# HKU-BAL/ClairS-TO

Measured on AMD Instinct MI355X. Metric: candidate sites/sec (pileup-tensor + AFF/NEG inference) at 1/2/4/8 MI355X, higher is better.
Workload: dtype f32; 1 GPU; ONT 50x synthetic pileups, SNV (K=4), 1M-site job cut into 4096-site chunks (BASELINE.json configs[1]); step = featurize(AFF+NEG) + CvT + BiGRU + posterior on one chunk; batch=4096, chunks_resident_per_gpu=16, min_bq_aff=20, pack_bytes_per_chunk=28614435, parallelism=sites sharded, 1 rank/GPU, weights=seeded random init (no pretrained weights offline)

## Files before the change

### clairs_to_amd/csrc/cvt_block.h

```cpp
#pragma once
#include "cvt_gemm.h"

namespace cto {

__host__ __device__ constexpr int emb_ps(int cin) { return cin > 0 ? ((cin - 4 + 15) / 16) * 16 + 4 : 0; }
__host__ __device__ constexpr int emb_kch(int cin) { return (3 * emb_ps(cin) + 15) / 16; }

template <int C, int W, int WKV, int TS>
struct CvtBlockGeom {
    static constexpr int R = TS * W, RKV = TS * WKV;
    static constexpr int MT = (R + 15) / 16, MTKV = (RKV + 15) / 16;
    static constexpr int RS = C + 4, QS = 68, HC = (4 * C < 128 ? 4 * C : 128), US = HC + 4;
    static constexpr int OFF_Y = 0;
    static constexpr int OFF_YKV = OFF_Y + MT * 16 * RS;
    static constexpr int OFF_Q = OFF_YKV + MTKV * 16 * RS;
    static constexpr int OFF_K = OFF_Q + MT * 16 * QS;
    static constexpr int OFF_V = OFF_K + MTKV * 16 * QS;
    static constexpr int OFF_END = OFF_V + MTKV * 16 * QS;
    static constexpr int SCRATCH = OFF_END - OFF_YKV;
    static constexpr int U_FLOATS = MT * 16 * US;
    static constexpr int TOTAL = OFF_END + (U_FLOATS > SCRATCH ? U_FLOATS - SCRATCH : 0);
    static constexpr size_t LDS_BYTES = size_t(TOTAL) * sizeof(float);
    static constexpr int TMP_FLOATS = OFF_END - OFF_Q;
    static constexpr int ALIAS = TOTAL - OFF_YKV;
    static constexpr int KCH1 = (W * RS + 15) / 16;
    static constexpr int emb_floats(int cin) { return (MT * 32 + 4) * emb_ps(cin); }
    static constexpr bool HEAD_OK = (TS == 16) && (64 + head_lds_floats(6) <= ALIAS);
};

template <int C, int W, int WKV, int TS>
__host__ __device__ constexpr bool MT_EXACT() { return (TS * W) % 16 == 0 && (TS * WKV) % 16 == 0; }

constexpr int CVT_BLOCK_THREADS = 512;
constexpr int CVT_WAVES = CVT_BLOCK_THREADS / 64;

template <int N>
struct ColOwn {
    static constexpr int TILES = N / 16;
    static constexpr int NOWN = TILES < CVT_WAVES ? TILES : CVT_WAVES;
    static constexpr int MSPLIT = CVT_WAVES / NOWN;
    static constexpr int NTW = TILES / NOWN;
    static_assert(TILES * 16 == N && CVT_WAVES % NOWN == 0 && NTW * NOWN == TILES, "unsupported GEMM width");
};
template <int MTx, int MSPLIT>
struct MSplit {
    static constexpr int MTG = (MTx + MSPLIT - 1) / MSPLIT;
    static constexpr int FULL = MTx / MTG;
    static constexpr int LAST = MTx - FULL * MTG;
};
struct TileSpan { int tile0, mbase, mcount; };
template <int N, int MTx>
__device__ __forceinline__ TileSpan tile_span(int wave) {
    using O = ColOwn<N>;
    constexpr int MTG = MSplit<MTx, O::MSPLIT>::MTG;
    const int mb = (wave / O::NOWN) * MTG;
    const int left = MTx - mb;
    return TileSpan{(wave % O::NOWN) * O::NTW, mb, left < 0 ? 0 : (left > MTG ? MTG : left)};
}
template <int N, int MTx, int KCH>
__device__ __forceinline__ void gemm_span(const TileSpan& sp, const float* A, int lda, const float* const (&wrow)[ColOwn<N>::NTW],
                                          const BPre<ColOwn<N>::NTW>& pre,
                                          f32x4 (&acc)[MSplit<MTx, ColOwn<N>::MSPLIT>::MTG][ColOwn<N>::NTW], int j, int kg) {
    using S = MSplit<MTx, ColOwn<N>::MSPLIT>;
    constexpr int NTW = ColOwn<N>::NTW;
    const float* A0 = A + sp.mbase * 16 * lda;
    if (ColOwn<N>::MSPLIT == 1 || sp.mcount == S::MTG) {
        gemm_lds<S::MTG, NTW, KCH>(A0, lda, wrow, pre, acc, j, kg);
    } else if constexpr (S::LAST > 0) {
        if (sp.mcount == S::LAST) {
            f32x4 (&sub)[S::LAST][NTW] = reinterpret_cast<f32x4 (&)[S::LAST][NTW]>(acc);
            gemm_lds<S::LAST, NTW, KCH>(A0, lda, wrow, pre, sub, j, kg);
        }
    }
}

template <int N, int MTx, int KCH, bool F16>
__device__ __forceinline__ void gemm_span_split(const TileSpan& sp, const float* A, int lda, int klo,
                                                const unsigned short* const (&wrow)[ColOwn<N>::NTW],
                                                const BPreS<ColOwn<N>::NTW>& pre,
                                                f32x4 (&acc)[MSplit<MTx, ColOwn<N>::MSPLIT>::MTG][ColOwn<N>::NTW], int j, int kg) {
    using S = MSplit<MTx, ColOwn<N>::MSPLIT>;
    constexpr int NTW = ColOwn<N>::NTW;
    const float* A0 = A + sp.mbase * 16 * lda;
    if (ColOwn<N>::MSPLIT == 1 || sp.mcount == S::MTG) {
        gemm_lds_split<S::MTG, NTW, KCH, F16>(A0, lda, klo, wrow, pre, acc, j, kg);
    } else if constexpr (S::LAST > 0) {
        if (sp.mcount == S::LAST) {
            f32x4 (&sub)[S::LAST][NTW] = reinterpret_cast<f32x4 (&)[S::LAST][NTW]>(acc);
            gemm_lds_split<S::LAST, NTW, KCH, F16>(A0, lda, klo, wrow, pre, sub, j, kg);
        }
    }
}

template <int C, int W, int WKV, int TS>
__host__ __device__ constexpr int cvt_blocks_per_cu() {
    return CvtBlockGeom<C, W, WKV, TS>::LDS_BYTES * 3 <= 160 * 1024 ? 3 : (CvtBlockGeom<C, W, WKV, TS>::LDS_BYTES * 2 <= 160 * 1024 ? 2 : 1);
}

template <int C, int W, int WKV, int TS, int CIN, bool HEAD, int SPLIT = 0>
__global__ __launch_bounds__(CVT_BLOCK_THREADS, (2 * cvt_blocks_per_cu<C, W, WKV, TS>())) void k_cvt_block(float* __restrict__ h, CvtStageParams sp,
                                                                                                            HeadTailParams hp, int heads, int B) {
    using G = CvtBlockGeom<C, W, WKV, TS>;
    constexpr bool SP = SPLIT != 0, F16 = SPLIT == 1;
    static_assert(!SP || (C % 64 == 0 && MT_EXACT<C, W, WKV, TS>()), "split GEMMs: 32-wide k chunks, 16-byte LayerNorm pieces, no pad rows");
    using WPtr = std::conditional_t<SP, const unsigned short*, const float*>;
    static_assert(CIN == 0 || G::emb_floats(CIN) <= G::ALIAS, "stage input tile does not fit the free LDS");
    static_assert(!HEAD || G::HEAD_OK, "classifier tail needs a 16-site tile and room for its scratch");
    static_assert(G::MT * 16 * G::RS <= G::TMP_FLOATS, "LayerNorm staging tile does not fit the q|k|v region");
    constexpr int NT = CVT_BLOCK_THREADS, NWV = CVT_WAVES;
    constexpr int R = G::R, MT = G::MT, MTKV = G::MTKV, RKV = G::RKV, RS = G::RS, QS = G::QS, HC = G::HC, US = G::US;
    static_assert(C % 16 == 0 && C <= 128 && NT % C == 0, "channel count must be 16, 32, 64 or 128");
    using OC = ColOwn<C>;
    using OQ = ColOwn<64>;
    using OKV = ColOwn<128>;
    using OF = ColOwn<HC>;
    constexpr int MGC = MSplit<MT, OC::MSPLIT>::MTG, MGQ = MSplit<MT, OQ::MSPLIT>::MTG, MGF = MSplit<MT, OF::MSPLIT>::MTG;
    constexpr int NTC = OC::NTW, NTF = OF::NTW;
    static_assert(OQ::NTW == 1 && OKV::NTW == 1 && OKV::MSPLIT == 1, "q / kv tiles: one column tile per wave");
    extern __shared__ __attribute__((aligned(16))) float smem[];
    float* sy = smem + G::OFF_Y;
    float* sykv = smem + G::OFF_YKV;
    float* sq = smem + G::OFF_Q;
    float* sk = smem + G::OFF_K;
    float* sv = smem + G::OFF_V;
    float* stmp = smem + G::OFF_Q;
    float* su = smem + G::OFF_YKV;

    const int tid = threadIdx.x, lane = tid & 63, wave = tid >> 6, j = lane & 15, kg = lane >> 4;
    const TileSpan spc = tile_span<C, MT>(wave), spq = tile_span<64, MT>(wave), spf = tile_span<HC, MT>(wave);
    const int site0 = blockIdx.x * TS;
    const int nsite = min(TS, B - site0);
    const int rows_valid = nsite * W;
    const int inner = heads * 64;
    float* hg = h + int64_t(site0) * W * C;
    int nstamp = 0;
    long long* const prof = sp.blk[0].prof;
    auto stamp = [&]() { if (prof && blockIdx.x == 0 && tid == 0 && nstamp < 250) prof[nstamp++] = clock64(); };
    stamp();
    const CvtBlockParams& pe = sp.blk[0];


    constexpr int KE_ = CIN > 0 ? emb_kch(CIN) : 1;
    const float* we_r[NTC];
    BPre<NTC> pre_e;
    if constexpr (CIN > 0) {
#pragma unroll
        for (int nt = 0; nt < NTC; ++nt) we_r[nt] = pe.wembp + int64_t(spc.tile0 + nt) * (KE_ * FRAG_CS) + 4 * lane;
        pre_e = prefetch_b<NTC, KE_>(we_r);
    }
    if constexpr (HEAD) {
        for (int i = tid; i < MT * 16; i += NT) *reinterpret_cast<float4*>(sy + i * RS + C) = make_float4(0.f, 0.f, 0.f, 0.f);
    }
    if constexpr (CIN == 0) {
        constexpr int NIT = (MT * 16 * (C / 4) + NT - 1) / NT;
        float4 stage[NIT];
#pragma unroll
        for (int q = 0; q < NIT; ++q) {
            const int i = tid + q * NT, r = i / (C / 4), c4 = (i - r * (C / 4)) * 4;
            stage[q] = (i < MT * 16 * (C / 4) && r < rows_valid) ? *reinterpret_cast<const float4*>(hg + r * C + c4) : make_float4(0.f, 0.f, 0.f, 0.f);
        }
#pragma unroll
        for (int q = 0; q < NIT; ++q) {
            const int i = tid + q * NT, r = i / (C / 4), c4 = (i - r * (C / 4)) * 4;
            if (i < MT * 16 * (C / 4)) *reinterpret_cast<float4*>(sy + r * RS + c4) = stage[q];
        }
        for (int i = tid; i < (MTKV * 16 - RKV) * RS; i += NT) sykv[RKV * RS + i] = 0.f;
    } else {
        constexpr int WIN = 2 * W - 1, PS = emb_ps(CIN), NPOS = MT * 32 + 4, VW = (CIN % 4 == 0) ? 4 : 2, SLOTS = PS / VW;
        static_assert(CIN % 2 == 0, "stage input channels must be even");
        float* sin = smem + G::OFF_YKV;
        const float* xg = pe.xin + int64_t(site0) * WIN * CIN;
        constexpr int NIT = (NPOS * SLOTS + NT - 1) / NT;
        float4 stage[NIT];
#pragma unroll
        for (int q = 0; q < NIT; ++q) {
            const int i = tid + q * NT;
            const int pp = i / SLOTS, c = (i - pp * SLOTS) * VW;
            const int s = pp / (2 * W), pos = pp - s * 2 * W - 1;
            const bool ok = i < NPOS * SLOTS && pos >= 0 && s < nsite && c < CIN;
            float4 v = make_float4(0.f, 0.f, 0.f, 0.f);
            if (ok) {
                if (pe.xraw) {
                    const short* src = pe.xraw + (int64_t(site0 + s) * WIN + pos) * CIN + c;
                    if constexpr (VW == 4) { const uint2 w = *reinterpret_cast<const uint2*>(src); v.x = __uint_as_float(w.x); v.y = __uint_as_float(w.y); }
                    else v.x = __uint_as_float(*reinterpret_cast<const unsigned*>(src));
                } else {
                    const float* src = xg + (s * WIN + pos) * CIN + c;
                    if constexpr (VW == 4) v = *reinterpret_cast<const float4*>(src);
                    else { const float2 w2 = *reinterpret_cast<const float2*>(src); v.x = w2.x; v.y = w2.y; }
                }
            }
            stage[q] = v;
        }
        if (pe.xraw) {
            static_assert(TS <= 64, "one lane per site of the tile");
            double sc_lane = 1.0;
            if (lane < nsite) {
                const int depth = pe.xinfo[int64_t(site0 + lane) * 12 + 1 + pe.xwhich];
                if (pe.xcov > 0 && depth > pe.xcov) sc_lane = double(pe.xcov) / double(depth);
            }
            const int sc_lo = __double2loint(sc_lane), sc_hi = __double2hiint(sc_lane);
#pragma unroll
            for (int q = 0; q < NIT; ++q) {
                const int i = tid + q * NT;
                const int pp = i / SLOTS, sx = pp / (2 * W), pos = pp - sx * 2 * W - 1;
                const int from = sx < TS ? sx : 0;
                const double sc = __hiloint2double(__shfl(sc_hi, from), __shfl(sc_lo, from));
                if (i < NPOS * SLOTS && pos >= 0 && sx < nsite) {
                    const unsigned w0 = __float_as_uint(stage[q].x), w1 = __float_as_uint(stage[q].y);
                    stage[q].x = float(double(int(short(w0 & 0xffffu))) * sc);
                    stage[q].y = float(double(int(short(w0 >> 16))) * sc);
                    if constexpr (VW == 4) { stage[q].z = float(double(int(short(w1 & 0xffffu))) * sc); stage[q].w = float(double(int(short(w1 >> 16))) * sc); }
                }
            }
        }
#pragma unroll
        for (int q = 0; q < NIT; ++q) {
            const int i = tid + q * NT;
            const int pp = i / SLOTS, c = (i - pp * SLOTS) * VW;
            if (i < NPOS * SLOTS) {
                if constexpr (VW == 4) *reinterpret_cast<float4*>(sin + pp * PS + c) = stage[q];
                else *reinterpret_cast<float2*>(sin + pp * PS + c) = make_float2(stage[q].x, stage[q].y);
            }
        }
    }
    lds_barrier();

    auto layer_norm = [&](const float* src, float* dst, const float* g, const float* b, auto split_out) {
#if CTO_CVT_ABL == 2
        return;
#endif
        constexpr bool SPO = decltype(split_out)::value;
        constexpr int CPL = C / 16, NP = (MT * 16 + NWV * 4 - 1) / (NWV * 4);
        const int l16 = lane & 15, grp = lane >> 4;
        float gv[CPL], bv[CPL];
#pragma unroll
        for (int i = 0; i < CPL; ++i) { gv[i] = g[l16 * CPL + i]; bv[i] = b[l16 * CPL + i]; }
        float v[NP][CPL];
#pragma unroll
        for (int q = 0; q < NP; ++q) {
            const int r = min(q * NWV * 4 + wave * 4 + grp, MT * 16 - 1);
            const float* xr = src + r * RS + l16 * CPL;
            if constexpr (CPL % 4 == 0) {
#pragma unroll
                for (int i = 0; i < CPL; i += 4) {
                    const float4 t = *reinterpret_cast<const float4*>(xr + i);
                    v[q][i] = t.x; v[q][i + 1] = t.y; v[q][i + 2] = t.z; v[q][i + 3] = t.w;
                }
            } else {
#pragma unroll
                for (int i = 0; i < CPL; ++i) v[q][i] = xr[i];
            }
        }
        float inv[NP];
#pragma unroll
        for (int q = 0; q < NP; ++q) {
            float sum = 0.f;
#pragma unroll
            for (int i = 0; i < CPL; ++i) sum += v[q][i];
            sum = row16_sum(sum);
            const float mean = sum / float(C);
            float sq2 = 0.f;
#pragma unroll
            for (int i = 0; i < CPL; ++i) { v[q][i] -= mean; sq2 += v[q][i] * v[q][i]; }
            sq2 = row16_sum(sq2);
            inv[q] = 1.0f / (sqrtf(sq2 / float(C)) + 1e-5f);
        }
#pragma unroll
        for (int q = 0; q < NP; ++q) {
            const int r = q * NWV * 4 + wave * 4 + grp;
            if (r < MT * 16) {
                float* yr = dst + r * RS + l16 * CPL;
                if constexpr (SPO) {
                    static_assert(!SPO || CPL % 4 == 0, "split rows are written four channels at a time");
#pragma unroll
                    for (int i = 0; i < CPL; i += 4)
                        put_split4<F16>(dst + r * RS, C, l16 * CPL + i, v[q][i] * inv[q] * gv[i] + bv[i], v[q][i + 1] * inv[q] * gv[i + 1] + bv[i + 1],
                                        v[q][i + 2] * inv[q] * gv[i + 2] + bv[i + 2], v[q][i + 3] * inv[q] * gv[i + 3] + bv[i + 3]);
                } else if constexpr (CPL % 4 == 0) {
#pragma unroll
                    for (int i = 0; i < CPL; i += 4)
                        *reinterpret_cast<float4*>(yr + i) =
                            make_float4(v[q][i] * inv[q] * gv[i] + bv[i], v[q][i + 1] * inv[q] * gv[i + 1] + bv[i + 1],
                                        v[q][i + 2] * inv[q] * gv[i + 2] + bv[i + 2], v[q][i + 3] * inv[q] * gv[i + 3] + bv[i + 3]);
                } else {
#pragma unroll
                    for (int i = 0; i < CPL; ++i) yr[i] = v[q][i] * inv[q] * gv[i] + bv[i];
                }
            }
        }
    };

    if constexpr (CIN > 0) {
        constexpr int PS = emb_ps(CIN), KE = emb_kch(CIN);
        f32x4 acc_e[MGC][NTC];
#pragma unroll
        for (int mt = 0; mt < MGC; ++mt)
#pragma unroll
            for (int nt = 0; nt < NTC; ++nt) acc_e[mt][nt] = f32x4{0.f, 0.f, 0.f, 0.f};
        gemm_span<C, MT, KE>(spc, smem + G::OFF_YKV, 2 * PS, we_r, pre_e, acc_e, j, kg);
#pragma unroll
        for (int nt = 0; nt < NTC; ++nt) {
            const int col = (spc.tile0 + nt) * 16 + j;
            const float bv = pe.bemb[col];
#pragma unroll
            for (int mt = 0; mt < MGC; ++mt)
                if (mt < spc.mcount) {
#pragma unroll
                    for (int r = 0; r < 4; ++r) sy[((spc.mbase + mt) * 16 + 4 * kg + r) * RS + col] = acc_e[mt][nt][r] + bv;
                }
        }
        lds_barrier();
        for (int i = tid; i < (MTKV * 16 - RKV) * RS; i += NT) sykv[RKV * RS + i] = 0.f;
        layer_norm(sy, sy, pe.lng, pe.lnb, std::false_type{});
        lds_barrier();
    }

    f32x4 acc_f[MGC][NTC];
    for (int bi = 0; bi < sp.nblk; ++bi) {
    const CvtBlockParams& p = sp.blk[bi];
    stamp();
    f32x4 acc_o[MGC][NTC];
#pragma unroll
    for (int nt = 0; nt < NTC; ++nt) {
        const int col = (spc.tile0 + nt) * 16 + j;
        const float bv = p.bo[col];
#pragma unroll
        for (int mt = 0; mt < MGC; ++mt) {
            const int row0 = (spc.mbase + (mt < spc.mcount ? mt : 0)) * 16 + 4 * kg;
            if (bi == 0) {
#pragma unroll
                for (int r = 0; r < 4; ++r) acc_o[mt][nt][r] = sy[(row0 + r) * RS + col] + bv;
            } else {
#pragma unroll
                for (int r = 0; r < 4; ++r) acc_o[mt][nt][r] = acc_f[mt][nt][r] + bv;
            }
        }
    }
    layer_norm(sy, stmp, p.n0g, p.n0b, std::false_type{});
    lds_barrier();
    stamp();

#if CTO_CVT_ABL != 2
    {
        constexpr int NSLOT = NT / C;
        constexpr int PG = NSLOT > TS ? NSLOT / TS : 1;
        constexpr int SL = PG > 1 ? TS : NSLOT, NIT = (TS + SL - 1) / SL;
        constexpr int WQ = (W + PG - 1) / PG, WK = (WKV + PG - 1) / PG;
        const int c = tid % C, slot = tid / C, pg = slot / SL, s0 = slot - pg * SL;
        const int wlo = pg * WQ, whi = min(W, wlo + WQ), klo = pg * WK, khi = min(WKV, klo + WK);
        const float q0 = p.dwq[c * 3], q1 = p.dwq[c * 3 + 1], q2 = p.dwq[c * 3 + 2];
        const float k0 = p.dwkv[c * 3], k1 = p.dwkv[c * 3 + 1], k2 = p.dwkv[c * 3 + 2];
        const float qm = p.bnq[c], qi = p.bnq[C + c], qw = p.bnq[2 * C + c], qb = p.bnq[3 * C + c];
        const float km = p.bnkv[c], ki = p.bnkv[C + c], kw = p.bnkv[2 * C + c], kb = p.bnkv[3 * C + c];
        float y[NIT][W];
#pragma unroll
        for (int it = 0; it < NIT; ++it) {
            const int s = min(s0 + it * SL, TS - 1);
#pragma unroll
            for (int w = 0; w < W; ++w) y[it][w] = stmp[(s * W + w) * RS + c];
        }
#pragma unroll
        for (int it = 0; it < NIT; ++it) {
            const int s = s0 + it * SL;
            if (s < TS && pg < PG) {
#pragma unroll
                for (int w = 0; w < W; ++w) {
                    if (PG > 1 && (w < wlo || w >= whi)) continue;
                    const float l = w > 0 ? y[it][w - 1] : 0.f, r = w + 1 < W ? y[it][w + 1] : 0.f;
                    const float d = q0 * l + q1 * y[it][w] + q2 * r;
                    if constexpr (SP) put_split1<F16>(sy + (s * W + w) * RS, C, c, (d - qm) * qi * qw + qb);
                    else sy[(s * W + w) * RS + c] = (d - qm) * qi * qw + qb;
                }
#pragma unroll
                for (int wo = 0; wo < WKV; ++wo) {
                    if (PG > 1 && (wo < klo || wo >= khi)) continue;
                    const int w = 2 * wo;
                    const float l = w > 0 ? y[it][w - 1] : 0.f, r = w + 1 < W ? y[it][w + 1] : 0.f;
                    const float d = k0 * l + k1 * y[it][w] + k2 * r;
                    if constexpr (SP) put_split1<F16>(sykv + (s * WKV + wo) * RS, C, c, (d - km) * ki * kw + kb);
                    else sykv[(s * WKV + wo) * RS + c] = (d - km) * ki * kw + kb;
                }
            }
        }
    }
#endif
    lds_barrier();

    stamp();
    auto frag = [&](const float* w, const unsigned short* ws, int tile, int kch, int c0) -> WPtr {
        if constexpr (SP) return ws + (int64_t(tile) * kch + c0) * SPLIT_CS + 8 * lane;
        else return w + (int64_t(tile) * kch + c0) * FRAG_CS + 4 * lane;
    };
    constexpr int KD = SP ? 32 : 16;
    auto q_rows = [&](int hh, WPtr (&wr)[1]) { wr[0] = frag(p.wq, p.wq_s, hh * 4 + spq.tile0, C / KD, 0); };
    auto o_rows = [&](int hh, WPtr (&wr)[NTC]) {
#pragma unroll
        for (int nt = 0; nt < NTC; ++nt) wr[nt] = frag(p.wo, p.wo_s, spc.tile0 + nt, inner / KD, hh * (64 / KD));
    };
    auto w1_rows = [&](int cc, WPtr (&wr)[NTF]) {
#pragma unroll
        for (int nt = 0; nt < NTF; ++nt) wr[nt] = frag(p.w1, p.w1_s, cc * (HC / 16) + spf.tile0 + nt, C / KD, 0);
    };
    auto w2_rows = [&](int cc, WPtr (&wr)[NTC]) {
#pragma unroll
        for (int nt = 0; nt < NTC; ++nt) wr[nt] = frag(p.w2, p.w2_s, spc.tile0 + nt, 4 * C / KD, cc * (HC / KD));
    };
    WPtr wq_r[1];
    q_rows(0, wq_r);
    auto pre_q = prefetch_b<1, C / KD>(wq_r);
    for (int hh = 0; hh < heads; ++hh) {
        const int wn = wave & 3;
        WPtr wkv1_r[1] = {frag(p.wkv, p.wkv_s, (wave < 4 ? 0 : inner / 16) + hh * 4 + wn, C / KD, 0)};
        const auto pre_kv1 = prefetch_b<1, C / KD>(wkv1_r);
        {
            f32x4 aq[MGQ][1];
#pragma unroll
            for (int mt = 0; mt < MGQ; ++mt) aq[mt][0] = f32x4{0.f, 0.f, 0.f, 0.f};
            if constexpr (SP) gemm_span_split<64, MT, C / 32, F16>(spq, sy, RS, C, wq_r, pre_q, aq, j, kg);
            else gemm_span<64, MT, C / 16>(spq, sy, RS, wq_r, pre_q, aq, j, kg);
#pragma unroll
            for (int mt = 0; mt < MGQ; ++mt)
                if (mt < spq.mcount) {
#pragma unroll
                    for (int r = 0; r < 4; ++r) sq[((spq.mbase + mt) * 16 + 4 * kg + r) * QS + spq.tile0 * 16 + j] = aq[mt][0][r];
                }
        }
        WPtr wo_r[NTC];
        o_rows(hh, wo_r);
        const auto pre_o = prefetch_b<NTC, 64 / KD>(wo_r);
        {
            f32x4 akv1[MTKV][1];
#pragma unroll
            for (int mt = 0; mt < MTKV; ++mt) akv1[mt][0] = f32x4{0.f, 0.f, 0.f, 0.f};
            if constexpr (SP) gemm_lds_split<MTKV, 1, C / 32, F16>(sykv, RS, C, wkv1_r, pre_kv1, akv1, j, kg);
            else gemm_lds<MTKV, 1, C / 16>(sykv, RS, wkv1_r, pre_kv1, akv1, j, kg);
            float* dst = wave < 4 ? sk : sv;
#pragma unroll
            for (int mt = 0; mt < MTKV; ++mt)
#pragma unroll
                for (int r = 0; r < 4; ++r) dst[(mt * 16 + 4 * kg + r) * QS + wn * 16 + j] = akv1[mt][0][r];
        }
        lds_barrier();
        stamp();
#if CTO_CVT_ABL != 2
        {
            constexpr int NPA = (R + NT / 16 - 1) / (NT / 16); constexpr int UF = WKV <= 5 ? 2 : 1;
            const int l4 = (lane & 15) * 4;
#pragma unroll UF
            for (int q = 0; q < NPA; ++q) {
                const int row = q * (NT / 16) + (tid >> 4);
                const int rr = row < R ? row : 0;
                const int s = rr / W;
                const float4 qv = *reinterpret_cast<const float4*>(sq + rr * QS + l4);
                float4 kv[WKV], vv[WKV];
#pragma unroll
                for (int jj = 0; jj < WKV; ++jj) {
                    kv[jj] = *reinterpret_cast<const float4*>(sk + (s * WKV + jj) * QS + l4);
                    vv[jj] = *reinterpret_cast<const float4*>(sv + (s * WKV + jj) * QS + l4);
                }
                float sc[WKV];
#pragma unroll
                for (int jj = 0; jj < WKV; ++jj) sc[jj] = fmaf(qv.w, kv[jj].w, fmaf(qv.z, kv[jj].z, fmaf(qv.y, kv[jj].y, qv.x * kv[jj].x)));
#pragma unroll
                for (int jj = 0; jj < WKV; ++jj) sc[jj] = row16_sum(sc[jj]);
                float mx = sc[0];
#pragma unroll
                for (int jj = 1; jj < WKV; ++jj) mx = fmaxf(mx, sc[jj]);
                float sum = 0.f;
#pragma unroll
                for (int jj = 0; jj < WKV; ++jj) { sc[jj] = exp_le0((sc[jj] - mx) * 0.125f); sum += sc[jj]; }
                float inv = rcp_fast(sum);
                inv = fmaf(fmaf(-sum, inv, 1.0f), inv, inv);
                float4 o4 = make_float4(0.f, 0.f, 0.f, 0.f);
#pragma unroll
                for (int jj = 0; jj < WKV; ++jj) {
                    const float pj = sc[jj] * inv;
                    o4.x = fmaf(pj, vv[jj].x, o4.x); o4.y = fmaf(pj, vv[jj].y, o4.y); o4.z = fmaf(pj, vv[jj].z, o4.z); o4.w = fmaf(pj, vv[jj].w, o4.w);
                }
                if (row < R) {
                    if constexpr (SP) put_split4<F16>(sq + rr * QS, 64, l4, o4.x, o4.y, o4.z, o4.w);
                    else *reinterpret_cast<float4*>(sq + rr * QS + l4) = o4;
                }
            }
        }
#endif
        if (hh + 1 < heads) {
            q_rows(hh + 1, wq_r);
            pre_q = prefetch_b<1, C / KD>(wq_r);
        }
        lds_barrier();
        stamp();
        if constexpr (SP) gemm_span_split<C, MT, 2, F16>(spc, sq, QS, 64, wo_r, pre_o, acc_o, j, kg);
        else gemm_span<C, MT, 4>(spc, sq, QS, wo_r, pre_o, acc_o, j, kg);
        lds_barrier();
        stamp();
    }

    WPtr w1_r[NTF];
    w1_rows(0, w1_r);
    auto pre_w1 = prefetch_b<NTF, C / KD>(w1_r);

#pragma unroll
    for (int nt = 0; nt < NTC; ++nt) {
        const int col = (spc.tile0 + nt) * 16 + j;
        const float bv = p.b2[col];
#pragma unroll
        for (int mt = 0; mt < MGC; ++mt) {
            if (mt < spc.mcount) {
#pragma unroll
                for (int r = 0; r < 4; ++r) stmp[((spc.mbase + mt) * 16 + 4 * kg + r) * RS + col] = acc_o[mt][nt][r];
            }
#pragma unroll
            for (int r = 0; r < 4; ++r) acc_f[mt][nt][r] = acc_o[mt][nt][r] + bv;
        }
    }
    lds_barrier();

    stamp();
    layer_norm(stmp, sy, p.n1g, p.n1b, std::bool_constant<SP>{});
    lds_barrier();
    stamp();

    for (int cc = 0; cc < 4 * C / HC; ++cc) {
        WPtr w2_r[NTC];
        w2_rows(cc, w2_r);
        const auto pre_w2 = prefetch_b<NTC, HC / KD>(w2_r);
        {
            f32x4 au[MGF][NTF];
#pragma unroll
            for (int mt = 0; mt < MGF; ++mt)
#pragma unroll
                for (int nt = 0; nt < NTF; ++nt) au[mt][nt] = f32x4{0.f, 0.f, 0.f, 0.f};
            if constexpr (SP) gemm_span_split<HC, MT, C / 32, F16>(spf, sy, RS, C, w1_r, pre_w1, au, j, kg);
            else gemm_span<HC, MT, C / 16>(spf, sy, RS, w1_r, pre_w1, au, j, kg);
            const int n0 = cc * HC + spf.tile0 * 16;
#pragma unroll
            for (int nt = 0; nt < NTF; ++nt) {
                const float bv = p.b1[n0 + nt * 16 + j];
#pragma unroll
                for (int mt = 0; mt < MGF; ++mt)
                    if (mt < spf.mcount) {
#pragma unroll
                        for (int r = 0; r < 4; ++r) {
                            float* urow = su + ((spf.mbase + mt) * 16 + 4 * kg + r) * US;
                            if constexpr (SP) put_split1<F16>(urow, HC, (spf.tile0 + nt) * 16 + j, gelu_f(au[mt][nt][r] + bv));
#if CTO_CVT_ABL == 2
                            else urow[(spf.tile0 + nt) * 16 + j] = au[mt][nt][r] + bv;
#else
                            else urow[(spf.tile0 + nt) * 16 + j] = gelu_f(au[mt][nt][r] + bv);
#endif
                        }
                    }
            }
        }
        if (cc + 1 < 4 * C / HC) {
            w1_rows(cc + 1, w1_r);
            pre_w1 = prefetch_b<NTF, C / KD>(w1_r);
        }
        lds_barrier();
        if constexpr (SP) gemm_span_split<C, MT, HC / 32, F16>(spc, su, US, HC, w2_r, pre_w2, acc_f, j, kg);
        else gemm_span<C, MT, HC / 16>(spc, su, US, w2_r, pre_w2, acc_f, j, kg);
        if (cc + 1 < 4 * C / HC) lds_barrier();
        stamp();
    }

#pragma unroll
    for (int nt = 0; nt < NTC; ++nt) {
        const int col = (spc.tile0 + nt) * 16 + j;
#pragma unroll
        for (int mt = 0; mt < MGC; ++mt)
            if (mt < spc.mcount) {
#pragma unroll
                for (int r = 0; r < 4; ++r) sy[((spc.mbase + mt) * 16 + 4 * kg + r) * RS + col] = acc_f[mt][nt][r];
            }
    }
    if (bi + 1 < sp.nblk) {
        lds_barrier();
        if constexpr (MTKV * 16 > RKV)
            for (int i = tid; i < (MTKV * 16 - RKV) * RS; i += NT) sykv[RKV * RS + i] = 0.f;
    }
    }
    const CvtBlockParams& p = sp.blk[sp.nblk - 1];
    if constexpr (!HEAD) {
        lds_barrier();
        for (int i = tid; i < rows_valid * (C / 4); i += NT) {
            const int r = i / (C / 4), c4 = (i - r * (C / 4)) * 4;
            *reinterpret_cast<float4*>(hg + r * C + c4) = *reinterpret_cast<const float4*>(sy + r * RS + c4);
        }
    }
    if constexpr (HEAD) {
        constexpr int K1 = G::KCH1;
        float* t1 = smem + G::OFF_YKV + 64;
        float* t2 = t1 + 16 * HEAD_T1S;
        const float* w1_r1[1] = {p.w1p + int64_t(wave) * (K1 * 256) + 4 * lane};
        BGroup<1, 7> g0;
        load_group<1, K1, 7, 256>(g0, w1_r1, 0);
        lds_barrier();
        stamp();
        f32x4 a1[2][1] = {{f32x4{0.f, 0.f, 0.f, 0.f}}, {f32x4{0.f, 0.f, 0.f, 0.f}}};
        HeadPre hpre;
        gemm_m1<1, K1, 7, 256>(sy, W * RS, w1_r1, g0, a1, j, kg, [&] { head_prefetch(hpre, hp); });
        const float bv = p.b1h[wave * 16 + j];
#pragma unroll
        for (int r = 0; r < 4; ++r) t1[(4 * kg + r) * HEAD_T1S + wave * 16 + j] = selu_fast(a1[0][0][r] + a1[1][0][r] + bv);
        lds_barrier();
        stamp();
        head_tail(t1, t2, hp, B, site0, nsite, hpre);
    }
    stamp();
}

}
```

### clairs_to_amd/csrc/cvt_gemm.h

```cpp
constexpr int FRAG_CS = 256;
#pragma once
#ifndef CTO_CVT_ABL
#define CTO_CVT_ABL 0
#endif
#include <type_traits>
#include "nn_kernels.h"
#include "split_mfma.h"

namespace cto {

struct CvtBlockParams {
    const float *n0g, *n0b, *dwq, *bnq, *wq, *dwkv, *bnkv, *wkv, *wo, *bo, *n1g, *n1b, *w1, *b1, *w2, *b2;
    long long* prof;
    const float *xin, *wembp, *bemb, *lng, *lnb;
    const float *w1p, *b1h;
    const unsigned short *wq_s, *wkv_s, *wo_s, *w1_s, *w2_s;
    const short* xraw;
    const int* xinfo;
    int xwhich, xcov;
};

constexpr int CVT_MAX_BLK = 4;
struct CvtStageParams {
    CvtBlockParams blk[CVT_MAX_BLK];
    int nblk;
};

template <int NTW>
struct BPre {
    float4 b0[NTW], b1[NTW];
};
template <int NTW, int KCH>
__device__ __forceinline__ BPre<NTW> prefetch_b(const float* const (&wrow)[NTW]) {
    BPre<NTW> p;
#pragma unroll
    for (int nt = 0; nt < NTW; ++nt) {
        p.b0[nt] = ldg4(wrow[nt]);
        p.b1[nt] = KCH > 1 ? ldg4(wrow[nt] + FRAG_CS) : make_float4(0.f, 0.f, 0.f, 0.f);
    }
    return p;
}

template <int MT, int NTW, int KCH>
__device__ __forceinline__ void gemm_lds(const float* __restrict__ A, int lda, const float* const (&wrow)[NTW],
                                         const BPre<NTW>& pre, f32x4 (&acc)[MT][NTW], int j, int kg) {
#if CTO_CVT_ABL == 1
    return;
#endif
    float4 Bq[3][NTW];
#pragma unroll
    for (int nt = 0; nt < NTW; ++nt) { Bq[0][nt] = pre.b0[nt]; Bq[1][nt] = pre.b1[nt]; }
    float4 a[2][MT];
    const float* Arow = A + j * lda + 4 * kg;
#pragma unroll
    for (int mt = 0; mt < MT; ++mt) a[0][mt] = *reinterpret_cast<const float4*>(Arow + mt * 16 * lda);
#pragma unroll
    for (int c = 0; c < KCH; ++c) {
        if (c + 2 < KCH) {
#pragma unroll
            for (int nt = 0; nt < NTW; ++nt) Bq[(c + 2) % 3][nt] = ldg4(wrow[nt] + (c + 2) * FRAG_CS);
        }
        if (c + 1 < KCH) {
#pragma unroll
            for (int mt = 0; mt < MT; ++mt) a[(c + 1) & 1][mt] = *reinterpret_cast<const float4*>(Arow + mt * 16 * lda + (c + 1) * 16);
        }
        __builtin_amdgcn_sched_barrier(0);
#pragma unroll
        for (int e = 0; e < 4; ++e) {
#pragma unroll
            for (int nt = 0; nt < NTW; ++nt) {
                const float4 b4 = Bq[c % 3][nt];
                const float bv = e == 0 ? b4.x : (e == 1 ? b4.y : (e == 2 ? b4.z : b4.w));
#pragma unroll
                for (int mt = 0; mt < MT; ++mt) {
                    const float4 a4 = a[c & 1][mt];
                    const float av = e == 0 ? a4.x : (e == 1 ? a4.y : (e == 2 ? a4.z : a4.w));
                    acc[mt][nt] = mfma16(av, bv, acc[mt][nt]);
                }
            }
        }
        __builtin_amdgcn_sched_barrier(0);
    }
}

constexpr int SPLIT_LO = 512, SPLIT_CS = 1024;
template <int NTW>
struct BPreS {
    uint4 b[2][NTW][2];
};
template <int NTW, int KCH>
__device__ __forceinline__ BPreS<NTW> prefetch_b(const unsigned short* const (&wrow)[NTW]) {
    BPreS<NTW> p;
#pragma unroll
    for (int nt = 0; nt < NTW; ++nt)
#pragma unroll
        for (int c = 0; c < 2; ++c) {
            if (c < KCH) { p.b[c][nt][0] = ldg16(wrow[nt] + c * SPLIT_CS); p.b[c][nt][1] = ldg16(wrow[nt] + SPLIT_LO + c * SPLIT_CS); }
            else { p.b[c][nt][0] = make_uint4(0u, 0u, 0u, 0u); p.b[c][nt][1] = make_uint4(0u, 0u, 0u, 0u); }
        }
    return p;
}
template <int MT, int NTW, int KCH, bool F16>
__device__ __forceinline__ void gemm_lds_split(const float* __restrict__ A, int lda, int klo, const unsigned short* const (&wrow)[NTW],
                                               const BPreS<NTW>& pre, f32x4 (&acc)[MT][NTW], int j, int kg) {
    uint4 Bq[3][NTW][2];
#pragma unroll
    for (int nt = 0; nt < NTW; ++nt)
#pragma unroll
        for (int p = 0; p < 2; ++p) { Bq[0][nt][p] = pre.b[0][nt][p]; Bq[1][nt][p] = pre.b[1][nt][p]; }
    constexpr bool ADB = MT <= 5;
    uint4 a[ADB ? 2 : 1][MT][2];
    const unsigned short* Arow = reinterpret_cast<const unsigned short*>(A + j * lda) + 8 * kg;
    auto load_a = [&](int buf, int c) {
#pragma unroll
        for (int mt = 0; mt < MT; ++mt)
#pragma unroll
            for (int p = 0; p < 2; ++p)
                a[buf][mt][p] = *reinterpret_cast<const uint4*>(Arow + mt * 16 * lda * 2 + p * klo + c * 32);
    };
    if (ADB) load_a(0, 0);
#pragma unroll
    for (int c = 0; c < KCH; ++c) {
        if (c + 2 < KCH) {
#pragma unroll
            for (int nt = 0; nt < NTW; ++nt) {
                Bq[(c + 2) % 3][nt][0] = ldg16(wrow[nt] + (c + 2) * SPLIT_CS);
                Bq[(c + 2) % 3][nt][1] = ldg16(wrow[nt] + SPLIT_LO + (c + 2) * SPLIT_CS);
            }
        }
        if (ADB) { if (c + 1 < KCH) load_a((c + 1) & 1, c + 1); }
        else load_a(0, c);
        __builtin_amdgcn_sched_barrier(0);
#pragma unroll
        for (int pass = 0; pass < 3; ++pass) {
            const int pa = pass == 1 ? 1 : 0, pw = pass == 2 ? 1 : 0;
#pragma unroll
            for (int nt = 0; nt < NTW; ++nt)
#pragma unroll
                for (int mt = 0; mt < MT; ++mt) acc[mt][nt] = mfma_split<F16>(a[ADB ? (c & 1) : 0][mt][pa], Bq[c % 3][nt][pw], acc[mt][nt]);
        }
        __builtin_amdgcn_sched_barrier(0);
    }
}

template <int NTW, int DEPTH>
struct BGroup {
    float4 b[DEPTH][NTW];
};
template <int NTW, int KCH, int DEPTH, int CS = 16>
__device__ __forceinline__ void load_group(BGroup<NTW, DEPTH>& g, const float* const (&wrow)[NTW], int c0) {
#pragma unroll
    for (int d = 0; d < DEPTH; ++d)
#pragma unroll
        for (int nt = 0; nt < NTW; ++nt)
            if (c0 + d < KCH) g.b[d][nt] = ldg4(wrow[nt] + (c0 + d) * CS);
}
template <int NTW, int KCH, int DEPTH>
__device__ __forceinline__ void mfma_group(const BGroup<NTW, DEPTH>& g, const float* Arow, int c0, f32x4 (&acc)[2][NTW]) {
    float4 a[DEPTH];
#pragma unroll
    for (int d = 0; d < DEPTH; ++d)
        if (c0 + d < KCH) a[d] = *reinterpret_cast<const float4*>(Arow + (c0 + d) * 16);
#pragma unroll
    for (int d = 0; d < DEPTH; ++d) {
        if (c0 + d >= KCH) break;
#pragma unroll
        for (int e = 0; e < 4; ++e) {
            const float av = e == 0 ? a[d].x : (e == 1 ? a[d].y : (e == 2 ? a[d].z : a[d].w));
#pragma unroll
            for (int nt = 0; nt < NTW; ++nt) {
                const float4 b4 = g.b[d][nt];
                const float bv = e == 0 ? b4.x : (e == 1 ? b4.y : (e == 2 ? b4.z : b4.w));
                acc[d & 1][nt] = mfma16(av, bv, acc[d & 1][nt]);
            }
        }
    }
}
template <int NTW, int KCH, int DEPTH, int CS, typename F>
__device__ __forceinline__ void gemm_m1(const float* __restrict__ A, int lda, const float* const (&wrow)[NTW],
                                        const BGroup<NTW, DEPTH>& first, f32x4 (&acc)[2][NTW], int j, int kg, F&& under_last) {
    constexpr int NG = (KCH + DEPTH - 1) / DEPTH;
    const float* Arow = A + j * lda + 4 * kg;
    BGroup<NTW, DEPTH> g[3];
    g[0] = first;
    if (NG > 1) load_group<NTW, KCH, DEPTH, CS>(g[1], wrow, DEPTH);
    if (NG <= 2) under_last();
#pragma unroll
    for (int i = 0; i < NG; ++i) {
        if (i + 2 < NG) {
            load_group<NTW, KCH, DEPTH, CS>(g[(i + 2) % 3], wrow, (i + 2) * DEPTH);
            if (i + 3 == NG) under_last();
        }
        __builtin_amdgcn_sched_barrier(0);
        mfma_group<NTW, KCH, DEPTH>(g[i % 3], Arow, i * DEPTH, acc);
        __builtin_amdgcn_sched_barrier(0);
    }
}
template <int NTW, int KCH, int DEPTH>
__device__ __forceinline__ void gemm_m1(const float* __restrict__ A, int lda, const float* const (&wrow)[NTW],
                                        const BGroup<NTW, DEPTH>& first, f32x4 (&acc)[2][NTW], int j, int kg) {
    gemm_m1<NTW, KCH, DEPTH, 16>(A, lda, wrow, first, acc, j, kg, [] {});
}

struct HeadTailParams {
    const float *w2, *b2;
    const float *w3, *b3;
    float* logits;
    int K;
};
constexpr int HEAD_T1S = 132;
__host__ __device__ constexpr int head_t2s(int K) { return K * 128 + 4; }
__host__ __device__ constexpr int head_lds_floats(int K) { return 16 * HEAD_T1S + 16 * head_t2s(K); }

struct HeadPre {
    BGroup<2, 8> g[2];
};
__device__ __forceinline__ void head_prefetch(HeadPre& hpre, const HeadTailParams& hp) {
    const int tid = threadIdx.x, lane = tid & 63, wave = tid >> 6;
    const float* w0 = hp.w2 + int64_t(wave) * (8 * 256) + 4 * lane;
#pragma unroll
    for (int pi = 0; pi < 2; ++pi) {
        const float* wr[2] = {w0 + pi * 2 * 128 * 128, w0 + (pi * 2 + 1) * 128 * 128};
        load_group<2, 8, 8, 256>(hpre.g[pi], wr, 0);
    }
}

template <int K>
__device__ __forceinline__ void head_tail_k(const float* t1, float* t2, const HeadTailParams& hp, int64_t B, int64_t site0,
                                            int nsite, HeadPre& hpre) {
    const int tid = threadIdx.x, lane = tid & 63, wave = tid >> 6, j = lane & 15, kg = lane >> 4;
    constexpr int T2S = head_t2s(K);
    static_assert(K % 2 == 0 && K >= 4, "heads are processed in pairs; two pairs arrive prefetched");
    const float* wr[2];
    wr[0] = hp.w2 + int64_t(wave) * (8 * 256) + 4 * lane;
    wr[1] = wr[0] + 128 * 128;
    const float* Arow = t1 + j * HEAD_T1S + 4 * kg;
#pragma unroll
    for (int pi = 0; pi < K / 2; ++pi) {
        f32x4 acc[2][2];
#pragma unroll
        for (int a = 0; a < 2; ++a)
#pragma unroll
            for (int q = 0; q < 2; ++q) acc[a][q] = f32x4{0.f, 0.f, 0.f, 0.f};
        mfma_group<2, 8, 8>(hpre.g[pi & 1], Arow, 0, acc);
        __builtin_amdgcn_sched_barrier(0);
        if (pi + 2 < K / 2) {
            const float* wn[2] = {wr[0] + (pi + 2) * 2 * 128 * 128, wr[1] + (pi + 2) * 2 * 128 * 128};
            load_group<2, 8, 8, 256>(hpre.g[pi & 1], wn, 0);
        }
#pragma unroll
        for (int q = 0; q < 2; ++q) {
            const int col = (pi * 2 + q) * 128 + wave * 16 + j;
            const float bv = hp.b2[col];
#pragma unroll
            for (int r = 0; r < 4; ++r) t2[(4 * kg + r) * T2S + col] = selu_fast(acc[0][q][r] + acc[1][q][r] + bv);
        }
    }
    __syncthreads();
    const int part = tid & 3;
    for (int idx = tid >> 2; idx < 16 * K * 2; idx += blockDim.x >> 2) {
        const int site = idx / (2 * K), rem = idx - site * 2 * K, hh = rem >> 1, o = rem & 1;
        const float4* u = reinterpret_cast<const float4*>(t2 + site * T2S + hh * 128 + part * 32);
        const float4* w = reinterpret_cast<const float4*>(hp.w3 + (hh * 2 + o) * 128 + part * 32);
        float sum = 0.f;
#pragma unroll
        for (int i = 0; i < 8; ++i) {
            const float4 a = u[i], b = w[i];
            sum = fmaf(a.x, b.x, sum); sum = fmaf(a.y, b.y, sum); sum = fmaf(a.z, b.z, sum); sum = fmaf(a.w, b.w, sum);
        }
        sum += __shfl_xor(sum, 1, 4);
        sum += __shfl_xor(sum, 2, 4);
        if (part == 0 && site < nsite) hp.logits[(int64_t(hh) * B + site0 + site) * 2 + o] = selu_f(sum + hp.b3[hh * 2 + o]);
    }
}
__device__ __forceinline__ void head_tail(const float* t1, float* t2, const HeadTailParams& hp, int64_t B, int64_t site0,
                                          int nsite, HeadPre& hpre) {
    if (hp.K == 4) head_tail_k<4>(t1, t2, hp, B, site0, nsite, hpre);
    else head_tail_k<6>(t1, t2, hp, B, site0, nsite, hpre);
}

__global__ __launch_bounds__(512) void k_head(const float* __restrict__ slabs, int S, int64_t slab_stride,
                                              const float* __restrict__ b1, HeadTailParams hp, int64_t B) {
    extern __shared__ __attribute__((aligned(16))) float smem[];
    float* t1 = smem;
    float* t2 = smem + 16 * HEAD_T1S;
    const int64_t site0 = int64_t(blockIdx.x) * 16;
    const int nsite = int(min(int64_t(16), B - site0));
    HeadPre hpre;
    head_prefetch(hpre, hp);
    {
        const int site = threadIdx.x >> 5, c4 = (threadIdx.x & 31) * 4;
        float4 v = make_float4(0.f, 0.f, 0.f, 0.f);
        if (site < nsite) {
            for (int z = 0; z < S; ++z) {
                const float4 a = *reinterpret_cast<const float4*>(slabs + z * slab_stride + (site0 + site) * 128 + c4);
                v.x += a.x; v.y += a.y; v.z += a.z; v.w += a.w;
            }
        }
        const float4 bb = *reinterpret_cast<const float4*>(b1 + c4);
        *reinterpret_cast<float4*>(t1 + site * HEAD_T1S + c4) =
            make_float4(selu_fast(v.x + bb.x), selu_fast(v.y + bb.y), selu_fast(v.z + bb.z), selu_fast(v.w + bb.w));
    }
    lds_barrier();
    head_tail(t1, t2, hp, B, site0, nsite, hpre);
}


}
```

### clairs_to_amd/csrc/models.hip

```cpp
#include <cmath>
#include <cstdlib>
#include <cstring>
#include <map>
#include <memory>
#include <string>
#include <vector>
#include "common.h"
#include "nn_kernels.h"
#include "cvt_block.h"

using namespace cto;

int launch_gru_layer1(hipStream_t s, const float* x, const float* Wf, const float* bias, float* out, int64_t B);
int launch_gru_layer1_raw(hipStream_t s, const int16_t* x_raw, const int32_t* site_info, int which, int min_rescale_cov, const float* Wf,
                          const float* bias, float* out, int64_t B);
int launch_gru_layer2_fc1_split(hipStream_t s, const float* x, const void* Wp, const float* bias, const void* Fp, float* fc1_part,
                                int64_t B, bool f16, const float* scale5);
int launch_gru_layer1_split(hipStream_t s, const float* x, const void* Wp, const float* bias, float* out, int64_t B, bool f16,
                            const float* scale5);
int launch_gru_layer2_fc1(hipStream_t s, const float* x, const float* Wf, const float* bias, const float* fc1f, float* fc1_part, int64_t B);


struct cto_weights {
    std::map<std::string, std::vector<float>> t;
};

extern "C" cto_weights* cto_weights_new(void) { return new cto_weights(); }
extern "C" void cto_weights_free(cto_weights* w) { delete w; }
extern "C" int cto_weights_add(cto_weights* w, const char* name, const float* data, int64_t numel) {
    CTO_REQUIRE(w && name && data && numel >= 0, CTO_EINVAL, "cto_weights_add: bad argument");
    w->t[name].assign(data, data + numel);
    return CTO_OK;
}

namespace {

struct Arena {
    std::vector<void*> ptrs;
    ~Arena() { for (void* p : ptrs) (void)hipFree(p); }
    int alloc(void** out, size_t bytes) {
        CTO_HIP(hipMalloc(out, bytes ? bytes : 16));
        ptrs.push_back(*out);
        return CTO_OK;
    }
    int upload(const std::vector<float>& v, float** out) {
        void* p = nullptr;
        int rc = alloc(&p, v.size() * sizeof(float));
        if (rc != CTO_OK) return rc;
        CTO_HIP(hipMemcpy(p, v.data(), v.size() * sizeof(float), hipMemcpyHostToDevice));
        *out = static_cast<float*>(p);
        return CTO_OK;
    }
};

struct HeadDev {
    float *w1 = nullptr, *b1 = nullptr;
    float* w1p = nullptr;
    float *w2 = nullptr, *b2 = nullptr;
    float *w3 = nullptr, *b3 = nullptr;
    int k1 = 0;
};

struct BlockDev {
    float *n0g, *n0b, *dwq, *bnq, *wq, *dwkv, *bnkv, *wkv, *wo, *bo, *n1g, *n1b, *w1, *b1, *w2, *b2;
    float *wq_f = nullptr, *wkv_f = nullptr, *wo_f = nullptr, *w1_f = nullptr, *w2_f = nullptr;
    float *wq_s = nullptr, *wkv_s = nullptr, *wo_s = nullptr, *w1_s = nullptr, *w2_s = nullptr;
};

struct StageDev {
    int cin, c, win, w, wkv, heads, inner;
    float *wemb, *bemb, *lng, *lnb;
    float* wembp = nullptr;
    std::vector<BlockDev> blocks;
};

}

struct cto_model {
    int device = -1;
    int kind = 0;
    int n_out = 4;
    Arena arena;
    StageDev st[3];
    float *gb1 = nullptr, *gb2 = nullptr;
    float *gw1f = nullptr, *gw2f = nullptr, *f1f = nullptr;
    float *gw1_split = nullptr, *gw2_split = nullptr, *f1_split = nullptr;
    bool split_f16 = false;
    float split_sc1[5] = {1.f, 1.f, 1.f, 1.f, 1.f}, split_sc2[5] = {1.f, 1.f, 1.f, 1.f, 1.f};
    int cvt_split = 0;
    HeadDev head;
    int64_t macs = 0;
    int64_t ws_B = 0;
    std::vector<void*> ws_ptrs;
    float* b_xexp = nullptr;
    int64_t xexp_B = 0;
    bool fuse_blocks = true;
    bool fuse_embed = true;
    bool fuse_head = true;
    bool prof = false;
    bool prof_all = false;
    std::vector<std::pair<hipEvent_t, hipEvent_t>> prof_ev;
    std::vector<std::pair<hipEvent_t, hipEvent_t>> prof_ev1;
    int64_t prof_macs = 0;
    float *b_h = nullptr, *b_t = nullptr, *b_yq = nullptr, *b_ykv = nullptr, *b_q = nullptr, *b_kv = nullptr,
          *b_o = nullptr, *b_u = nullptr, *b_slab = nullptr, *b_h2 = nullptr;
    ~cto_model() {
        if (b_xexp) (void)hipFree(b_xexp);
        for (void* p : ws_ptrs) (void)hipFree(p);
        for (auto& e : prof_ev) { (void)hipEventDestroy(e.first); (void)hipEventDestroy(e.second); }
        for (auto& e : prof_ev1) { (void)hipEventDestroy(e.first); (void)hipEventDestroy(e.second); }
    }
};

namespace {

const std::vector<float>* find(const cto_weights* w, const std::string& name, int64_t numel, int* rc) {
    auto it = w->t.find(name);
    if (it == w->t.end()) { set_error("weight '%s' missing", name.c_str()); *rc = CTO_EMISSING; return nullptr; }
    if (int64_t(it->second.size()) != numel) {
        set_error("weight '%s' has %zu elements, expected %lld", name.c_str(), it->second.size(), (long long)numel);
        *rc = CTO_EMISSING;
        return nullptr;
    }
    return &it->second;
}

#define GETW(var, name, numel)                                   \
    const std::vector<float>* var = find(w, (name), (numel), &rc); \
    if (!var) return rc;

std::vector<float> pack_fragments(const float* W, int ntiles, int kch) {
    std::vector<float> f(size_t(ntiles) * kch * 256);
    for (int t = 0; t < ntiles; ++t)
        for (int c = 0; c < kch; ++c)
            for (int lane = 0; lane < 64; ++lane) {
                const int j = lane & 15, kg = lane >> 4;
                for (int e = 0; e < 4; ++e)
                    f[((size_t(t) * kch + c) * 64 + lane) * 4 + e] = W[size_t(t * 16 + j) * (kch * 16) + c * 16 + 4 * kg + e];
            }
    return f;
}

int build_head(const cto_weights* w, const char* const* names, int K, int k1, const std::vector<float>* w1perm,
               Arena& a, HeadDev& h) {
    int rc = CTO_OK;
    h.k1 = k1;
    GETW(b1, "fc1.bias", 128);
    if (w1perm && (rc = a.upload(*w1perm, &h.w1)) != CTO_OK) return rc;
    if ((rc = a.upload(*b1, &h.b1)) != CTO_OK) return rc;
    std::vector<float> w2(size_t(K) * 128 * 128), b2(size_t(K) * 128), w3(size_t(K) * 2 * 128), b3(size_t(K) * 2);
    for (int k = 0; k < K; ++k) {
        const std::string p = names[k];
        GETW(f2w, p + "_fc2.weight", 128 * 128);
        GETW(f2b, p + "_fc2.bias", 128);
        GETW(f3w, p + "_fc3.weight", 2 * 128);
        GETW(f3b, p + "_fc3.bias", 2);
        const std::vector<float> frag = pack_fragments(f2w->data(), 8, 8);
        std::copy(frag.begin(), frag.end(), w2.begin() + size_t(k) * 128 * 128);
        std::copy(f2b->begin(), f2b->end(), b2.begin() + size_t(k) * 128);
        std::copy(f3w->begin(), f3w->end(), w3.begin() + size_t(k) * 256);
        std::copy(f3b->begin(), f3b->end(), b3.begin() + size_t(k) * 2);
    }
    if ((rc = a.upload(w2, &h.w2)) != CTO_OK) return rc;
    if ((rc = a.upload(b2, &h.b2)) != CTO_OK) return rc;
    if ((rc = a.upload(w3, &h.w3)) != CTO_OK) return rc;
    if ((rc = a.upload(b3, &h.b3)) != CTO_OK) return rc;
    return CTO_OK;
}

int pack_bn(const cto_weights* w, const std::string& p, int C, Arena& a, float** out) {
    int rc = CTO_OK;
    GETW(wt, p + ".weight", C);
    GETW(bs, p + ".bias", C);
    GETW(mu, p + ".running_mean", C);
    GETW(var, p + ".running_var", C);
    std::vector<float> v(size_t(4) * C);
    for (int c = 0; c < C; ++c) {
        v[size_t(c)] = (*mu)[size_t(c)];
        v[size_t(C + c)] = float(1.0 / std::sqrt(double((*var)[size_t(c)]) + 1e-5));
        v[size_t(2 * C + c)] = (*wt)[size_t(c)];
        v[size_t(3 * C + c)] = (*bs)[size_t(c)];
    }
    return a.upload(v, out);
}

int pack_dw(const cto_weights* w, const std::string& name, int C, Arena& a, float** out) {
    int rc = CTO_OK;
    GETW(k, name, int64_t(C) * 9);
    std::vector<float> v(size_t(C) * 3);
    for (int c = 0; c < C; ++c)
        for (int t = 0; t < 3; ++t) v[size_t(c * 3 + t)] = (*k)[size_t((c * 3 + 1) * 3 + t)];
    return a.upload(v, out);
}

int upload_named(const cto_weights* w, const std::string& name, int64_t numel, Arena& a, float** out) {
    int rc = CTO_OK;
    GETW(v, name, numel);
    return a.upload(*v, out);
}

int launch_gemm(hipStream_t s, const float* A, int64_t lda, const float* W, int64_t ldw, const float* bias,
                const float* R, int64_t ldr, float* C, int64_t ldc, int M, int N, int K, int act,
                int conv_win = 0, int conv_wout = 0, int conv_cin = 0, int splitk = 1, int64_t slab = 0) {
    GemmArgs g;
    g.A = A; g.lda = lda; g.W = W; g.ldw = ldw; g.bias = bias; g.R = R; g.ldr = ldr; g.C = C; g.ldc = ldc;
    g.M = M; g.N = N; g.K = K; g.act = act;
    g.conv_win = conv_win; g.conv_wout = conv_wout; g.conv_cin = conv_cin;
    g.kslice = splitk > 1 ? int(cdiv(cdiv(K, splitk), 16) * 16) : K;
    g.slab = slab;
    g.vecA = (conv_wout == 0 && (lda % 4) == 0 && (K % 4) == 0 && (reinterpret_cast<uintptr_t>(A) % 16) == 0) ? 1 : 0;
    if (M <= 0) return CTO_OK;
    if (N <= 16) {
        dim3 grid(unsigned(cdiv(M, 128)), unsigned(cdiv(N, 16)), unsigned(splitk));
        hipLaunchKernelGGL((k_gemm<4, 1, 2, 1>), grid, dim3(256), 0, s, g);
    } else if (N <= 64) {
        dim3 grid(unsigned(cdiv(M, 64)), unsigned(cdiv(N, 64)), unsigned(splitk));
        hipLaunchKernelGGL((k_gemm<2, 2, 2, 2>), grid, dim3(256), 0, s, g);
    } else {
        dim3 grid(unsigned(cdiv(M, 64)), unsigned(cdiv(N, 128)), unsigned(splitk));
        hipLaunchKernelGGL((k_gemm<2, 2, 2, 4>), grid, dim3(256), 0, s, g);
    }
    CTO_HIP(hipGetLastError());
    return CTO_OK;
}

int ensure_ws(cto_model* m, int64_t B) {
    if (B <= m->ws_B) return CTO_OK;
    for (void* p : m->ws_ptrs) (void)hipFree(p);
    m->ws_ptrs.clear();
    m->ws_B = 0;
    auto get = [&](float** out, int64_t per_site) -> int {
        void* p = nullptr;
        CTO_HIP(hipMalloc(&p, size_t(B) * size_t(per_site) * sizeof(float)));
        m->ws_ptrs.push_back(p);
        *out = static_cast<float*>(p);
        return CTO_OK;
    };
    int rc;
    if (m->kind == 0) {
        int64_t act = 0, qn = 0, kvn = 0, un = 0;
        for (const StageDev& s : m->st) {
            act = std::max<int64_t>(act, int64_t(s.w) * s.c);
            qn = std::max<int64_t>(qn, int64_t(s.w) * s.inner);
            kvn = std::max<int64_t>(kvn, int64_t(s.wkv) * 2 * s.inner);
            un = std::max<int64_t>(un, int64_t(s.w) * 4 * s.c);
        }
        if ((rc = get(&m->b_h, act)) || (rc = get(&m->b_h2, act)) || (rc = get(&m->b_t, act)) || (rc = get(&m->b_yq, act)) ||
            (rc = get(&m->b_ykv, act)) || (rc = get(&m->b_q, qn)) || (rc = get(&m->b_kv, kvn)) ||
            (rc = get(&m->b_o, qn)) || (rc = get(&m->b_u, un)) || (rc = get(&m->b_slab, 4 * 128)))
            return rc;
    } else {
        if ((rc = get(&m->b_h, 33 * 256)) || (rc = get(&m->b_slab, 2 * 128))) return rc;
    }
    m->ws_B = B;
    return CTO_OK;
}

int launch_head(cto_model* m, hipStream_t s, const float* slabs, int S, int64_t B, float* logits) {
    const HeadDev& h = m->head;
    const int K = m->n_out;
    const size_t smem = size_t(head_lds_floats(K)) * sizeof(float);
    static bool attr_set = false;
    if (!attr_set) {
        CTO_HIP(hipFuncSetAttribute(reinterpret_cast<const void*>(&k_head), hipFuncAttributeMaxDynamicSharedMemorySize,
                                    int(head_lds_floats(6) * sizeof(float))));
        attr_set = true;
    }
    HeadTailParams hp{h.w2, h.b2, h.w3, h.b3, logits, K};
    hipLaunchKernelGGL(k_head, dim3(unsigned(cdiv(B, 16))), dim3(512), smem, s, slabs, S, B * 128, h.b1, hp, B);
    CTO_HIP(hipGetLastError());
    return CTO_OK;
}

int run_head(cto_model* m, hipStream_t s, const float* feat, int64_t B, float* logits) {
    const HeadDev& h = m->head;
    int rc;
    if (feat == nullptr)
        return launch_head(m, s, m->b_slab, 2, B, logits);
    const int S = 4;
    if ((rc = launch_gemm(s, feat, h.k1, h.w1, h.k1, nullptr, nullptr, 0, m->b_slab, 128, int(B), 128, h.k1, ACT_NONE,
                          0, 0, 0, S, B * 128)))
        return rc;
    return launch_head(m, s, m->b_slab, S, B, logits);
}

struct RawIn { const int16_t* x; const int32_t* site_info; int which, min_rescale_cov; };

struct BlockExtra {
    const float* xin = nullptr;
    const RawIn* raw = nullptr;
    const StageDev* st = nullptr;
    const HeadDev* head = nullptr;
    float* logits = nullptr;
    int n_out = 0;
};

template <int C, int W, int WKV, int TS, int CIN, bool HEAD, int SPLIT = 0>
int launch_cvt_block(hipStream_t s, float* h, const BlockDev* blocks, int nblk, int heads, int64_t B, const BlockExtra& ex) {
    using G = CvtBlockGeom<C, W, WKV, TS>;
    static_assert(G::LDS_BYTES <= 160 * 1024, "fused CvT block does not fit the 160 KB LDS of a gfx950 CU");
    static bool attr_set = false;
    if (!attr_set) {
        CTO_HIP(hipFuncSetAttribute(reinterpret_cast<const void*>(&k_cvt_block<C, W, WKV, TS, CIN, HEAD, SPLIT>),
                                    hipFuncAttributeMaxDynamicSharedMemorySize, int(G::LDS_BYTES)));
        attr_set = true;
    }
    static long long* prof_buf = nullptr;
    static const bool prof_on = [] { const char* e = getenv("CTO_BLOCK_PROF"); return e && e[0] == '1'; }();
    if (prof_on && !prof_buf) CTO_HIP(hipMalloc(reinterpret_cast<void**>(&prof_buf), 256 * sizeof(long long)));
    if (prof_on) CTO_HIP(hipMemsetAsync(prof_buf, 0, 256 * sizeof(long long), s));
    CvtStageParams sp{};
    sp.nblk = nblk;
    for (int i = 0; i < nblk; ++i) {
        const BlockDev& b = blocks[i];
        sp.blk[i] = CvtBlockParams{b.n0g, b.n0b, b.dwq, b.bnq, b.wq_f, b.dwkv, b.bnkv, b.wkv_f, b.wo_f, b.bo, b.n1g, b.n1b, b.w1_f, b.b1, b.w2_f, b.b2,
                                   prof_on ? prof_buf : nullptr, nullptr, nullptr, nullptr, nullptr, nullptr, nullptr, nullptr,
                                   nullptr, nullptr, nullptr, nullptr, nullptr};
        if (SPLIT != 0) {
            CTO_REQUIRE(b.wq_s && b.wkv_s && b.wo_s && b.w1_s && b.w2_s, CTO_EINVAL, "split CvT block without split weights");
            CvtBlockParams& p = sp.blk[i];
            p.wq_s = reinterpret_cast<const unsigned short*>(b.wq_s); p.wkv_s = reinterpret_cast<const unsigned short*>(b.wkv_s);
            p.wo_s = reinterpret_cast<const unsigned short*>(b.wo_s); p.w1_s = reinterpret_cast<const unsigned short*>(b.w1_s);
            p.w2_s = reinterpret_cast<const unsigned short*>(b.w2_s);
        }
    }
    HeadTailParams hp{};
    if (CIN > 0) {
        CvtBlockParams& p = sp.blk[0];
        p.xin = ex.xin; p.wembp = ex.st->wembp; p.bemb = ex.st->bemb; p.lng = ex.st->lng; p.lnb = ex.st->lnb;
        if (ex.raw) { p.xraw = reinterpret_cast<const short*>(ex.raw->x); p.xinfo = ex.raw->site_info; p.xwhich = ex.raw->which; p.xcov = ex.raw->min_rescale_cov; }
    }
    if (HEAD) {
        CvtBlockParams& p = sp.blk[nblk - 1];
        p.w1p = ex.head->w1p; p.b1h = ex.head->b1;
        hp = HeadTailParams{ex.head->w2, ex.head->b2, ex.head->w3, ex.head->b3, ex.logits, ex.n_out};
    }
    hipLaunchKernelGGL((k_cvt_block<C, W, WKV, TS, CIN, HEAD, SPLIT>), dim3(unsigned(cdiv(B, TS))), dim3(CVT_BLOCK_THREADS), G::LDS_BYTES,
                       s, h, sp, hp, heads, int(B));
    CTO_HIP(hipGetLastError());
    if (prof_on) {
        long long hst[256];
        CTO_HIP(hipStreamSynchronize(s));
        CTO_HIP(hipMemcpy(hst, prof_buf, sizeof(hst), hipMemcpyDeviceToHost));
        fprintf(stderr, "k_cvt_block<%d,%d,%d,%d,%d,%d> x%d stamps:", C, W, WKV, TS, CIN, int(HEAD), nblk);
        for (int i = 1; i < 256 && hst[i]; ++i) fprintf(stderr, " %lld", hst[i] - hst[i - 1]);
        fprintf(stderr, "\n");
    }
    return CTO_OK;
}

template <int C, int W, int WKV, int TS, int CIN, int SPLIT>
int dispatch_block_kind(hipStream_t s, float* h, const BlockDev* blocks, int nblk, int heads, int64_t B, const BlockExtra& ex, bool embed, bool head) {
    if constexpr (C == 128 && CvtBlockGeom<C, W, WKV, TS>::HEAD_OK) {
        if (head) return embed ? launch_cvt_block<C, W, WKV, TS, CIN, true, SPLIT>(s, h, blocks, nblk, heads, B, ex)
                               : launch_cvt_block<C, W, WKV, TS, 0, true, SPLIT>(s, h, blocks, nblk, heads, B, ex);
    }
    return embed ? launch_cvt_block<C, W, WKV, TS, CIN, false, SPLIT>(s, h, blocks, nblk, heads, B, ex)
                 : launch_cvt_block<C, W, WKV, TS, 0, false, SPLIT>(s, h, blocks, nblk, heads, B, ex);
}
template <int C, int W, int WKV, int TS, int CIN>
int dispatch_block(hipStream_t s, float* h, const BlockDev* blocks, int nblk, int heads, int64_t B, const BlockExtra& ex, bool embed, bool head,
                   int split) {
    if constexpr (C % 64 == 0 && MT_EXACT<C, W, WKV, TS>()) {
        if (split == 1) return dispatch_block_kind<C, W, WKV, TS, CIN, 1>(s, h, blocks, nblk, heads, B, ex, embed, head);
        if (split == 2) return dispatch_block_kind<C, W, WKV, TS, CIN, 2>(s, h, blocks, nblk, heads, B, ex, embed, head);
    }
    return dispatch_block_kind<C, W, WKV, TS, CIN, 0>(s, h, blocks, nblk, heads, B, ex, embed, head);
}
#ifndef CTO_CVT_TS1
#define CTO_CVT_TS1 8
#endif
#ifndef CTO_CVT_TS2
#define CTO_CVT_TS2 16
#endif
#ifndef CTO_CVT_TS3
#define CTO_CVT_TS3 16
#endif
struct FusedGeom { int c, w, wkv, ts, cin; };
const FusedGeom* fused_geom(const StageDev& st) {
    static const FusedGeom G[4] = {{128, 5, 3, CTO_CVT_TS3, 64}, {64, 9, 5, CTO_CVT_TS2, 16}, {16, 17, 9, CTO_CVT_TS1, 34}, {32, 17, 9, CTO_CVT_TS1, 34}};
    for (const FusedGeom& g : G)
        if (st.c == g.c && st.w == g.w && st.wkv == g.wkv) return &g;
    return nullptr;
}
bool can_fuse_embed(const StageDev& st) { const FusedGeom* g = fused_geom(st); return g && g->cin == st.cin && st.wembp; }
bool can_fuse_head(const StageDev& st, const HeadDev& hd) { const FusedGeom* g = fused_geom(st); return g && g->ts == 16 && g->c == 128 && hd.w1p; }

int try_fused_blocks(hipStream_t s, const StageDev& st, const BlockDev* b, int nblk, float* h, int64_t B, const BlockExtra& ex, bool embed,
                     bool head, int split) {
    int rc = CTO_OK;
    if (!b->wq_s) split = 0;
    if (st.c == 128 && st.w == 5 && st.wkv == 3) rc = dispatch_block<128, 5, 3, CTO_CVT_TS3, 64>(s, h, b, nblk, st.heads, B, ex, embed, head, split);
    else if (st.c == 64 && st.w == 9 && st.wkv == 5) rc = dispatch_block<64, 9, 5, CTO_CVT_TS2, 16>(s, h, b, nblk, st.heads, B, ex, embed, head, split);
    else if (st.c == 16 && st.w == 17 && st.wkv == 9) rc = dispatch_block<16, 17, 9, CTO_CVT_TS1, 34>(s, h, b, nblk, st.heads, B, ex, embed, head, split);
    else if (st.c == 32 && st.w == 17 && st.wkv == 9) rc = dispatch_block<32, 17, 9, CTO_CVT_TS1, 34>(s, h, b, nblk, st.heads, B, ex, embed, head, split);
    else return 0;
    return rc == CTO_OK ? 1 : rc;
}

int cvt_forward(cto_model* m, const float* x, int64_t B, float* logits, hipStream_t s, const RawIn* raw = nullptr) {
    int rc;
    const float* in = x;
    for (int si = 0; si < 3; ++si) {
        const StageDev& st = m->st[si];
        const int M = int(B) * st.w, Mkv = int(B) * st.wkv, C = st.c;
        float* hbuf = (si & 1) ? m->b_h2 : m->b_h;
        const bool embed_in_block = m->fuse_blocks && m->fuse_embed && can_fuse_embed(st);
        if (!embed_in_block) {
            if ((rc = launch_gemm(s, in, 0, st.wemb, 3 * st.cin, st.bemb, nullptr, 0, m->b_t, C, M, C, 3 * st.cin, ACT_NONE,
                                  st.win, st.w, st.cin)))
                return rc;
            hipLaunchKernelGGL(k_layernorm, dim3(unsigned(cdiv(M, 4))), dim3(256), 0, s, m->b_t, hbuf, st.lng, st.lnb, M, C);
            CTO_HIP(hipGetLastError());
        }
        static const int group_max = [] {
            const char* e = getenv("CTO_CVT_BLOCKS_PER_LAUNCH");
            const int v = e ? atoi(e) : CVT_MAX_BLK;
            return v < 1 ? 1 : (v > CVT_MAX_BLK ? CVT_MAX_BLK : v);
        }();
        for (size_t bi = 0; bi < st.blocks.size(); ++bi) {
            const BlockDev& b = st.blocks[bi];
            if (m->fuse_blocks) {
                BlockExtra ex;
                const int nblk = int(std::min<size_t>(size_t(group_max), st.blocks.size() - bi));
                const bool embed = embed_in_block && bi == 0;
                const bool head = m->fuse_head && si == 2 && bi + size_t(nblk) == st.blocks.size() && can_fuse_head(st, m->head);
                ex.xin = in; ex.st = &st; ex.head = &m->head; ex.logits = logits; ex.n_out = m->n_out;
                ex.raw = (si == 0 && embed) ? raw : nullptr;
                const int fr = try_fused_blocks(s, st, &b, nblk, hbuf, B, ex, embed, head, m->cvt_split);
                if (fr < 0) return fr;
                if (fr == 1) {
                    if (head) return CTO_OK;
                    bi += size_t(nblk) - 1;
                    continue;
                }
            }
            float* h = hbuf;
            hipLaunchKernelGGL(k_ln_dw, dim3(unsigned(B)), dim3(256), 0, s, h, b.n0g, b.n0b, b.dwq, b.bnq, b.dwkv,
                               b.bnkv, m->b_yq, m->b_ykv, st.w, st.wkv, C);
            CTO_HIP(hipGetLastError());
            if ((rc = launch_gemm(s, m->b_yq, C, b.wq, C, nullptr, nullptr, 0, m->b_q, st.inner, M, st.inner, C, ACT_NONE)))
                return rc;
            if ((rc = launch_gemm(s, m->b_ykv, C, b.wkv, C, nullptr, nullptr, 0, m->b_kv, 2 * st.inner, Mkv, 2 * st.inner,
                                  C, ACT_NONE)))
                return rc;
            const size_t smem = size_t(st.w * st.inner + st.wkv * 2 * st.inner + st.heads * st.w * st.wkv) * sizeof(float);
            hipLaunchKernelGGL(k_attention, dim3(unsigned(B)), dim3(256), smem, s, m->b_q, m->b_kv, m->b_o, st.w, st.wkv,
                               st.heads);
            CTO_HIP(hipGetLastError());
            if ((rc = launch_gemm(s, m->b_o, st.inner, b.wo, st.inner, b.bo, h, C, h, C, M, C, st.inner, ACT_NONE)))
                return rc;
            hipLaunchKernelGGL(k_layernorm, dim3(unsigned(cdiv(M, 4))), dim3(256), 0, s, h, m->b_t, b.n1g, b.n1b, M, C);
            CTO_HIP(hipGetLastError());
            if ((rc = launch_gemm(s, m->b_t, C, b.w1, C, b.b1, nullptr, 0, m->b_u, 4 * C, M, 4 * C, C, ACT_GELU))) return rc;
            if ((rc = launch_gemm(s, m->b_u, 4 * C, b.w2, 4 * C, b.b2, h, C, h, C, M, C, 4 * C, ACT_NONE))) return rc;
        }
        in = hbuf;
    }
    return run_head(m, s, in, B, logits);
}

int prof_begin(hipStream_t s, hipEvent_t* e0, hipEvent_t* e1) {
    CTO_HIP(hipEventCreate(e0));
    CTO_HIP(hipEventCreate(e1));
    CTO_HIP(hipEventRecord(*e0, s));
    return CTO_OK;
}

int bigru_forward(cto_model* m, const float* x, int64_t B, float* logits, hipStream_t s, const RawIn* raw = nullptr) {
    int rc;
    hipEvent_t e0 = nullptr, e1 = nullptr;
    if (m->prof_all && (rc = prof_begin(s, &e0, &e1))) return rc;
    if (raw) rc = launch_gru_layer1_raw(s, raw->x, raw->site_info, raw->which, raw->min_rescale_cov, m->gw1f, m->gb1, m->b_h, B);
    else if (m->gw1_split) rc = launch_gru_layer1_split(s, x, m->gw1_split, m->gb1, m->b_h, B, m->split_f16, m->split_sc1);
    else rc = launch_gru_layer1(s, x, m->gw1f, m->gb1, m->b_h, B);
    if (rc) return rc;
    if (m->prof_all) {
        CTO_HIP(hipEventRecord(e1, s));
        m->prof_ev1.emplace_back(e0, e1);
    }
    if (m->prof && (rc = prof_begin(s, &e0, &e1))) return rc;
    if (m->gw2_split) rc = launch_gru_layer2_fc1_split(s, m->b_h, m->gw2_split, m->gb2, m->f1_split, m->b_slab, B, m->split_f16, m->split_sc2);
    else rc = launch_gru_layer2_fc1(s, m->b_h, m->gw2f, m->gb2, m->f1f, m->b_slab, B);
    if (rc) return rc;
    if (m->prof) {
        CTO_HIP(hipEventRecord(e1, s));
        m->prof_ev.emplace_back(e0, e1);
    }
    return run_head(m, s, nullptr, B, logits);
}

int pack_gru(const cto_weights* w, const std::string& base, int kin, int kp, int H, Arena& a, float** bout, float** Wfout) {
    int rc = CTO_OK;
    const int KT = kp + H;
    const int NB = H / 64, NX = kp / 16, NC = NX + H / 16;
    const bool tail1 = (kin % 16 != 0) && (kin - 16 * (NX - 1) <= 4);
    std::vector<float> W(size_t(2) * 3 * H * KT, 0.f), bv(size_t(2) * 4 * H), Wf(size_t(2) * 4 * NC * NB * 3 * 256, 0.f);
    for (int d = 0; d < 2; ++d) {
        const std::string sfx = d == 0 ? "" : "_reverse";
        GETW(wih, base + ".weight_ih_l0" + sfx, int64_t(3) * H * kin);
        GETW(whh, base + ".weight_hh_l0" + sfx, int64_t(3) * H * H);
        GETW(bih, base + ".bias_ih_l0" + sfx, 3 * H);
        GETW(bhh, base + ".bias_hh_l0" + sfx, 3 * H);
        for (int n = 0; n < 3 * H; ++n) {
            float* row = W.data() + (size_t(d) * 3 * H + n) * KT;
            for (int k = 0; k < kin; ++k) row[k] = (*wih)[size_t(n) * kin + k];
            for (int k = 0; k < H; ++k) row[kp + k] = (*whh)[size_t(n) * H + k];
        }
        for (int wv = 0; wv < 4; ++wv)
            for (int c = 0; c < NC; ++c)
                for (int nb = 0; nb < NB; ++nb)
                    for (int q = 0; q < 3; ++q)
                        for (int lane = 0; lane < 64; ++lane) {
                            const int jj = lane & 15, kg = lane >> 4;
                            const float* row = W.data() + (size_t(d) * 3 * H + q * H + (wv * NB + nb) * 16 + jj) * KT;
                            float* f = &Wf[(((((size_t(d) * 4 + wv) * NC + c) * NB + nb) * 3 + q) * 64 + lane) * 4];
                            if (tail1 && c == NX - 1) f[0] = row[16 * c + kg];
                            else for (int e = 0; e < 4; ++e) f[e] = row[16 * c + 4 * kg + e];
                        }
        float* b = bv.data() + size_t(d) * 4 * H;
        for (int j = 0; j < H; ++j) {
            b[0 * H + j] = (*bih)[size_t(j)] + (*bhh)[size_t(j)];
            b[1 * H + j] = (*bih)[size_t(H + j)] + (*bhh)[size_t(H + j)];
            b[2 * H + j] = (*bih)[size_t(2 * H + j)];
            b[3 * H + j] = (*bhh)[size_t(2 * H + j)];
        }
    }
    if ((rc = a.upload(Wf, Wfout)) != CTO_OK) return rc;
    return a.upload(bv, bout);
}

std::vector<float> pack_fc1_fragments(const std::vector<float>& fc1, int H) {
    const int T = 33, NH = H / 16;
    std::vector<float> f(size_t(2) * T * 4 * NH * 2 * 256);
    for (int d = 0; d < 2; ++d)
        for (int t = 0; t < T; ++t)
            for (int wv = 0; wv < 4; ++wv)
                for (int kh = 0; kh < NH; ++kh)
                    for (int nt = 0; nt < 2; ++nt)
                        for (int lane = 0; lane < 64; ++lane) {
                            const int jj = lane & 15, kg = lane >> 4;
                            const float* src = fc1.data() + size_t(wv * 32 + nt * 16 + jj) * (T * 2 * H) + size_t(t) * 2 * H + d * H + 16 * kh + 4 * kg;
                            float* dst = &f[((((((size_t(d) * T + t) * 4 + wv) * NH + kh) * 2 + nt) * 64) + lane) * 4];
                            for (int e = 0; e < 4; ++e) dst[e] = src[e];
                        }
    return f;
}

inline uint16_t bf16_rne(float v) {
    uint32_t u;
    memcpy(&u, &v, 4);
    return uint16_t((u + 0x7fffu + ((u >> 16) & 1u)) >> 16);
}
inline float bf16_value(uint16_t h) {
    const uint32_t u = uint32_t(h) << 16;
    float v;
    memcpy(&v, &u, 4);
    return v;
}
inline uint16_t f16_rne(float v) {
    const _Float16 h = _Float16(v);
    uint16_t u;
    memcpy(&u, &h, 2);
    return u;
}
inline float f16_value(uint16_t u) {
    _Float16 h;
    memcpy(&h, &u, 2);
    return float(h);
}
inline void put_split8(uint16_t* hi, uint16_t* lo, const float* src, int n_valid, bool f16, float scale = 1.f) {
    for (int e = 0; e < 8; ++e) {
        const float v = e < n_valid ? src[e] * scale : 0.f;
        if (f16) { hi[e] = f16_rne(v); lo[e] = f16_rne(v - f16_value(hi[e])); }
        else { hi[e] = bf16_rne(v); lo[e] = bf16_rne(v - bf16_value(hi[e])); }
    }
}
int upload_halves(const std::vector<uint16_t>& v, Arena& a, float** out) {
    std::vector<float> f(v.size() / 2);
    memcpy(f.data(), v.data(), v.size() * 2);
    return a.upload(f, out);
}
int upload_split_fragments(const cto_weights* w, const std::string& name, int ntiles, int kch32, bool f16, Arena& a, float** out) {
    int rc = CTO_OK;
    const int K = kch32 * 32;
    GETW(v, name, int64_t(ntiles) * 16 * K);
    std::vector<uint16_t> fr(size_t(ntiles) * kch32 * 2 * 64 * 8);
    for (int t = 0; t < ntiles; ++t)
        for (int c = 0; c < kch32; ++c)
            for (int lane = 0; lane < 64; ++lane) {
                const int j = lane & 15, kg = lane >> 4;
                const float* src = v->data() + size_t(t * 16 + j) * K + c * 32 + kg * 8;
                if (f16)
                    for (int e = 0; e < 8; ++e)
                        CTO_REQUIRE(std::fabs(src[e]) < 60000.f, CTO_EUNSUPPORTED, "CTO_CVT_SPLIT=f16: weight %s holds %g, outside the f16 range",
                                    name.c_str(), double(src[e]));
                const size_t u = ((size_t(t) * kch32 + c) * 2) * 64;
                put_split8(&fr[(u + lane) * 8], &fr[(u + 64 + lane) * 8], src, 8, f16);
            }
    return upload_halves(fr, a, out);
}
int upload_fragments(const cto_weights* w, const std::string& name, int ntiles, int kch, Arena& a, float** out) {
    int rc = CTO_OK;
    GETW(v, name, int64_t(ntiles) * 16 * kch * 16);
    return a.upload(pack_fragments(v->data(), ntiles, kch), out);
}

int pack_gru_split(const cto_weights* w, const std::string& base, int kin, int kp, int H, const std::vector<float>* fc1, bool f16,
                   int log2_sx, Arena& a, float** Wout, float** Fout, float* scale5) {
    const int NB = H / 64, NX = kp / 32, NH = H / 32, NC = NX + NH, T = 33;
    int rc = CTO_OK;
    std::vector<uint16_t> W(size_t(2) * 4 * NC * NB * 6 * 64 * 8), F(fc1 ? size_t(2) * T * 4 * NH * 4 * 64 * 8 : 0);
    float w_ih_scale = 1.f, w_hh_scale = 1.f, f_scale = 1.f;
    scale5[0] = scale5[1] = scale5[2] = scale5[3] = scale5[4] = 1.f;
    if (f16) {
        float mx_ih = 0.f, mx_hh = 0.f, mx_f = 0.f;
        for (int d = 0; d < 2; ++d) {
            const std::string sfx = d == 0 ? "" : "_reverse";
            GETW(wih, base + ".weight_ih_l0" + sfx, int64_t(3) * H * kin);
            GETW(whh, base + ".weight_hh_l0" + sfx, int64_t(3) * H * H);
            for (float v : *wih) mx_ih = std::max(mx_ih, std::fabs(v));
            for (float v : *whh) mx_hh = std::max(mx_hh, std::fabs(v));
        }
        if (fc1) for (float v : *fc1) mx_f = std::max(mx_f, std::fabs(v));
        CTO_REQUIRE(std::isfinite(mx_ih) && std::isfinite(mx_hh) && std::isfinite(mx_f), CTO_EUNSUPPORTED,
                    "split f16: %s holds a non-finite weight", base.c_str());
        auto room = [](float mx) { return mx > 0.f ? std::max(-60, std::min(60, int(std::floor(std::log2(32768.0 / double(mx)))))) : 60; };
        const int log2_sh = 14;
        const int S = std::min(log2_sx + room(mx_ih), log2_sh + room(mx_hh));
        w_ih_scale = std::ldexp(1.f, S - log2_sx);
        w_hh_scale = std::ldexp(1.f, S - log2_sh);
        const int Sf = room(mx_f);
        f_scale = std::ldexp(1.f, Sf);
        scale5[0] = std::ldexp(1.f, log2_sx); scale5[1] = std::ldexp(1.f, log2_sh); scale5[2] = std::ldexp(1.f, S);
        scale5[3] = std::ldexp(1.f, -S); scale5[4] = std::ldexp(1.f, -(log2_sh + Sf));
    }
    for (int d = 0; d < 2; ++d) {
        const std::string sfx = d == 0 ? "" : "_reverse";
        GETW(wih, base + ".weight_ih_l0" + sfx, int64_t(3) * H * kin);
        GETW(whh, base + ".weight_hh_l0" + sfx, int64_t(3) * H * H);
        for (int wv = 0; wv < 4; ++wv)
            for (int c = 0; c < NC; ++c)
                for (int nb = 0; nb < NB; ++nb)
                    for (int q = 0; q < 3; ++q)
                        for (int lane = 0; lane < 64; ++lane) {
                            const int j = lane & 15, kg = lane >> 4;
                            const int n = q * H + (wv * NB + nb) * 16 + j;
                            const int k0 = (c < NX ? c : c - NX) * 32 + kg * 8;
                            const float* src = c < NX ? wih->data() + size_t(n) * kin + k0 : whh->data() + size_t(n) * H + k0;
                            const int n_valid = c < NX ? std::max(0, std::min(8, kin - k0)) : 8;
                            const size_t u = ((((size_t(d) * 4 + wv) * NC + c) * NB + nb) * 6 + q * 2) * 64;
                            put_split8(&W[(u + lane) * 8], &W[(u + 64 + lane) * 8], n_valid > 0 ? src : whh->data(), n_valid, f16,
                                       c < NX ? w_ih_scale : w_hh_scale);
                        }
        for (int t = 0; fc1 && t < T; ++t)
            for (int wv = 0; wv < 4; ++wv)
                for (int kh = 0; kh < NH; ++kh)
                    for (int nt = 0; nt < 2; ++nt)
                        for (int lane = 0; lane < 64; ++lane) {
                            const int j = lane & 15, kg = lane >> 4;
                            const int n = wv * 32 + nt * 16 + j;
                            const float* src = fc1->data() + size_t(n) * (T * 2 * H) + size_t(t) * 2 * H + d * H + kh * 32 + kg * 8;
                            const size_t u = ((((size_t(d) * T + t) * 4 + wv) * NH + kh) * 4 + nt * 2) * 64;
                            put_split8(&F[(u + lane) * 8], &F[(u + 64 + lane) * 8], src, 8, f16, f_scale);
                        }
    }
    rc = upload_halves(W, a, Wout);
    return rc != CTO_OK || !fc1 ? rc : upload_halves(F, a, Fout);
}

}

extern "C" int cto_cvt_create(const cto_weights* w, const cto_cvt_cfg* cfg, cto_model** out) {
    return cto_cvt_create_ex(w, cfg, CTO_SPLIT_ENV, out);
}

extern "C" int cto_cvt_create_ex(const cto_weights* w, const cto_cvt_cfg* cfg, int split_mode, cto_model** out) {
    CTO_REQUIRE(w && cfg && out, CTO_EINVAL, "cto_cvt_create: null argument");
    CTO_REQUIRE(split_mode >= CTO_SPLIT_ENV && split_mode <= CTO_SPLIT_BF16, CTO_EINVAL, "cto_cvt_create_ex: split_mode %d", split_mode);
    CTO_REQUIRE(cfg->n_out == 4 || cfg->n_out == 6, CTO_EINVAL, "n_out must be 4 or 6");
    for (int i = 0; i < 3; ++i)
        CTO_REQUIRE(cfg->emb_dim[i] >= 4 && cfg->emb_dim[i] <= 128 && cfg->emb_dim[i] % 4 == 0 && cfg->heads[i] >= 1 &&
                        cfg->heads[i] <= 8 && cfg->depth[i] >= 1,
                    CTO_EUNSUPPORTED, "CvT stage %d config out of range (emb_dim <= 128, multiple of 4)", i + 1);
    std::unique_ptr<cto_model> m(new cto_model());
    CTO_HIP(hipGetDevice(&m->device));
    m->kind = 0;
    m->n_out = cfg->n_out;
    {
        const char* e = split_mode == CTO_SPLIT_ENV ? getenv("CTO_CVT_SPLIT") : nullptr;
        if (e && e[0]) {
            const std::string kind(e);
            CTO_REQUIRE(kind == "f16" || kind == "bf16", CTO_EINVAL, "CTO_CVT_SPLIT must be f16 or bf16, not '%s'", e);
            m->cvt_split = kind == "f16" ? 1 : 2;
        }
        if (split_mode > 0) m->cvt_split = split_mode;
    }
    Arena& a = m->arena;
    int rc = CTO_OK;
    int cin = CTO_NCHAN, win = CTO_NPOS;
    int64_t macs = 0;
    auto fail = [&](int code) { return code; };
    for (int si = 0; si < 3; ++si) {
        StageDev& st = m->st[si];
        st.cin = cin; st.c = cfg->emb_dim[si]; st.win = win; st.w = (win + 1) / 2; st.wkv = (st.w + 1) / 2;
        st.heads = cfg->heads[si]; st.inner = 64 * st.heads;
        const int C = st.c;
        const std::string L = "layer" + std::to_string(si + 1);
        {
            GETW(cw, L + ".0.weight", int64_t(C) * cin * 9);
            std::vector<float> v(size_t(C) * 3 * cin);
            for (int n = 0; n < C; ++n)
                for (int t = 0; t < 3; ++t)
                    for (int ci = 0; ci < cin; ++ci)
                        v[(size_t(n) * 3 + t) * cin + ci] = (*cw)[((size_t(n) * cin + ci) * 3 + 1) * 3 + t];
            if ((rc = a.upload(v, &st.wemb))) return fail(rc);
            const int PS = emb_ps(cin), KP = emb_kch(cin) * 16;
            std::vector<float> vp(size_t(C) * KP, 0.f);
            for (int n = 0; n < C; ++n)
                for (int t = 0; t < 3; ++t)
                    for (int ci = 0; ci < cin; ++ci) vp[size_t(n) * KP + t * PS + ci] = v[(size_t(n) * 3 + t) * cin + ci];
            if (C % 16 == 0) { if ((rc = a.upload(pack_fragments(vp.data(), C / 16, KP / 16), &st.wembp))) return fail(rc); }
        }
        if ((rc = upload_named(w, L + ".0.bias", C, a, &st.bemb))) return fail(rc);
        if ((rc = upload_named(w, L + ".1.g", C, a, &st.lng))) return fail(rc);
        if ((rc = upload_named(w, L + ".1.b", C, a, &st.lnb))) return fail(rc);
        macs += int64_t(st.w) * 3 * cin * C;
        for (int d = 0; d < cfg->depth[si]; ++d) {
            BlockDev b;
            const std::string P = L + ".2.layers." + std::to_string(d);
            if ((rc = upload_named(w, P + ".0.norm.g", C, a, &b.n0g)) || (rc = upload_named(w, P + ".0.norm.b", C, a, &b.n0b)) ||
                (rc = pack_dw(w, P + ".0.fn.to_q.net.0.weight", C, a, &b.dwq)) ||
                (rc = pack_bn(w, P + ".0.fn.to_q.net.1", C, a, &b.bnq)) ||
                (rc = upload_named(w, P + ".0.fn.to_q.net.2.weight", int64_t(st.inner) * C, a, &b.wq)) ||
                (rc = pack_dw(w, P + ".0.fn.to_kv.net.0.weight", C, a, &b.dwkv)) ||
                (rc = pack_bn(w, P + ".0.fn.to_kv.net.1", C, a, &b.bnkv)) ||
                (rc = upload_named(w, P + ".0.fn.to_kv.net.2.weight", int64_t(2) * st.inner * C, a, &b.wkv)) ||
                (rc = upload_named(w, P + ".0.fn.to_out.0.weight", int64_t(C) * st.inner, a, &b.wo)) ||
                (rc = upload_named(w, P + ".0.fn.to_out.0.bias", C, a, &b.bo)) ||
                (rc = upload_named(w, P + ".1.norm.g", C, a, &b.n1g)) || (rc = upload_named(w, P + ".1.norm.b", C, a, &b.n1b)) ||
                (rc = upload_named(w, P + ".1.fn.net.0.weight", int64_t(4) * C * C, a, &b.w1)) ||
                (rc = upload_named(w, P + ".1.fn.net.0.bias", 4 * C, a, &b.b1)) ||
                (rc = upload_named(w, P + ".1.fn.net.3.weight", int64_t(4) * C * C, a, &b.w2)) ||
                (rc = upload_named(w, P + ".1.fn.net.3.bias", C, a, &b.b2)))
                return fail(rc);
            const int NI = st.inner / 16, NC16 = C / 16;
            if (C % 16 == 0 &&
                ((rc = upload_fragments(w, P + ".0.fn.to_q.net.2.weight", NI, NC16, a, &b.wq_f)) ||
                (rc = upload_fragments(w, P + ".0.fn.to_kv.net.2.weight", 2 * NI, NC16, a, &b.wkv_f)) ||
                (rc = upload_fragments(w, P + ".0.fn.to_out.0.weight", NC16, NI, a, &b.wo_f)) ||
                (rc = upload_fragments(w, P + ".1.fn.net.0.weight", 4 * NC16, NC16, a, &b.w1_f)) ||
                 (rc = upload_fragments(w, P + ".1.fn.net.3.weight", NC16, 4 * NC16, a, &b.w2_f))))
                return fail(rc);
            if (m->cvt_split && C % 64 == 0) {
                const bool f16 = m->cvt_split == 1;
                if ((rc = upload_split_fragments(w, P + ".0.fn.to_q.net.2.weight", NI, C / 32, f16, a, &b.wq_s)) ||
                    (rc = upload_split_fragments(w, P + ".0.fn.to_kv.net.2.weight", 2 * NI, C / 32, f16, a, &b.wkv_s)) ||
                    (rc = upload_split_fragments(w, P + ".0.fn.to_out.0.weight", NC16, st.inner / 32, f16, a, &b.wo_s)) ||
                    (rc = upload_split_fragments(w, P + ".1.fn.net.0.weight", 4 * NC16, C / 32, f16, a, &b.w1_s)) ||
                    (rc = upload_split_fragments(w, P + ".1.fn.net.3.weight", NC16, 4 * C / 32, f16, a, &b.w2_s)))
                    return fail(rc);
            }
            st.blocks.push_back(b);
            macs += int64_t(st.w) * C * st.inner + int64_t(st.wkv) * C * 2 * st.inner + int64_t(st.w) * st.inner * C +
                    int64_t(st.w) * 8 * C * C + int64_t(2) * st.heads * st.w * st.wkv * 64 +
                    int64_t(3) * C * (st.w + st.wkv);
        }
        cin = C;
        win = st.w;
    }
    const int C3 = m->st[2].c, W3 = m->st[2].w, k1 = C3 * W3;
    {
        GETW(f1, "fc1.weight", int64_t(128) * k1);
        std::vector<float> v(size_t(128) * k1);
        for (int n = 0; n < 128; ++n)
            for (int c = 0; c < C3; ++c)
                for (int ww = 0; ww < W3; ++ww) v[size_t(n) * k1 + ww * C3 + c] = (*f1)[size_t(n) * k1 + c * W3 + ww];
        static const char* const names[6] = {"a", "c", "g", "t", "i", "d"};
        if ((rc = build_head(w, names, m->n_out, k1, &v, a, m->head))) return fail(rc);
        if (C3 == 128 && W3 == 5) {
            using G = CvtBlockGeom<128, 5, 3, 16>;
            const int KP = G::KCH1 * 16;
            std::vector<float> vp(size_t(128) * KP, 0.f);
            for (int n = 0; n < 128; ++n)
                for (int ww = 0; ww < W3; ++ww)
                    for (int c = 0; c < C3; ++c) vp[size_t(n) * KP + ww * G::RS + c] = v[size_t(n) * k1 + ww * C3 + c];
            if ((rc = a.upload(pack_fragments(vp.data(), 8, G::KCH1), &m->head.w1p))) return fail(rc);
        }
    }
    macs += int64_t(k1) * 128 + int64_t(m->n_out) * (128 * 128 + 256);
    m->macs = macs;
    if (const char* e = getenv("CTO_CVT_UNFUSED")) m->fuse_blocks = !(e[0] == '1');
    if (const char* e = getenv("CTO_CVT_NO_EMBED_FUSE")) m->fuse_embed = !(e[0] == '1');
    if (const char* e = getenv("CTO_CVT_NO_HEAD_FUSE")) m->fuse_head = !(e[0] == '1');
    *out = m.release();
    return CTO_OK;
}

extern "C" int cto_bigru_create(const cto_weights* w, int n_out, cto_model** out) {
    return cto_bigru_create_ex(w, n_out, CTO_SPLIT_ENV, out);
}

extern "C" int cto_bigru_create_ex(const cto_weights* w, int n_out, int split_mode, cto_model** out) {
    CTO_REQUIRE(w && out, CTO_EINVAL, "cto_bigru_create: null argument");
    CTO_REQUIRE(split_mode >= CTO_SPLIT_ENV && split_mode <= CTO_SPLIT_BF16, CTO_EINVAL, "cto_bigru_create_ex: split_mode %d", split_mode);
    CTO_REQUIRE(n_out == 4 || n_out == 6, CTO_EINVAL, "n_out must be 4 or 6");
    std::unique_ptr<cto_model> m(new cto_model());
    CTO_HIP(hipGetDevice(&m->device));
    m->kind = 1;
    m->n_out = n_out;
    int rc = CTO_OK;
    auto fail = [&](int code) { return code; };
    if ((rc = pack_gru(w, "lstm", 34, 48, 128, m->arena, &m->gb1, &m->gw1f))) return fail(rc);
    if ((rc = pack_gru(w, "lstm_2", 256, 256, 192, m->arena, &m->gb2, &m->gw2f))) return fail(rc);
    const int k1 = 33 * 384;
    {
        GETW(f1, "fc1.weight", int64_t(128) * k1);
        static const char* const names[6] = {"na", "nc", "ng", "nt", "ni", "nd"};
        if ((rc = build_head(w, names, n_out, k1, nullptr, m->arena, m->head))) return fail(rc);
        if ((rc = m->arena.upload(pack_fc1_fragments(*f1, 192), &m->f1f))) return fail(rc);
        const char* e = split_mode == CTO_SPLIT_ENV ? getenv("CTO_GRU_SPLIT") : split_mode == CTO_SPLIT_F16 ? "f16" : split_mode == CTO_SPLIT_BF16 ? "bf16" : nullptr;
        if (e && e[0]) {
            const std::string kind(e);
            CTO_REQUIRE(kind == "f16" || kind == "bf16", CTO_EINVAL, "CTO_GRU_SPLIT must be f16 or bf16, not '%s'", e);
            m->split_f16 = kind == "f16";
            if ((rc = pack_gru_split(w, "lstm_2", 256, 256, 192, f1, m->split_f16, 14, m->arena, &m->gw2_split, &m->f1_split, m->split_sc2))) return fail(rc);
            const char* l = getenv("CTO_GRU_SPLIT_LAYERS");
            if (!(l && l[0] == '2') && (rc = pack_gru_split(w, "lstm", 34, 64, 128, nullptr, m->split_f16, 0, m->arena, &m->gw1_split, nullptr, m->split_sc1)))
                return fail(rc);
        }
    }
    m->macs = int64_t(33) * 2 * 3 * 128 * (34 + 128) + int64_t(33) * 2 * 3 * 192 * (256 + 192) + int64_t(k1) * 128 +
              int64_t(n_out) * (128 * 128 + 256);
    *out = m.release();
    return CTO_OK;
}

namespace {
int forward_preamble(const char* fn, cto_model* m, bool args_ok, int64_t B) {
    CTO_REQUIRE(args_ok, CTO_EINVAL, "%s: bad argument", fn);
    CTO_REQUIRE(B * 33 < (int64_t(1) << 31) / 640, CTO_EUNSUPPORTED, "batch too large for 32-bit row indices; split it");
    if (B == 0) return CTO_OK;
    int dev = -1;
    CTO_HIP(hipGetDevice(&dev));
    CTO_REQUIRE(dev == m->device, CTO_EINVAL, "%s: model lives on device %d but device %d is current (one process per GPU)", fn, m->device, dev);
    return ensure_ws(m, B);
}

int cvt_forward_timed(cto_model* m, const float* x, int64_t B, float* logits, hipStream_t s, const RawIn* raw = nullptr) {
    int rc;
    hipEvent_t e0 = nullptr, e1 = nullptr;
    if (m->prof && (rc = prof_begin(s, &e0, &e1))) return rc;
    rc = cvt_forward(m, x, B, logits, s, raw);
    if (m->prof && rc == CTO_OK) {
        CTO_HIP(hipEventRecord(e1, s));
        m->prof_ev.emplace_back(e0, e1);
    }
    return rc;
}

__global__ __launch_bounds__(256) void k_expand_raw(const int16_t* __restrict__ raw, const int32_t* __restrict__ site_info, int which, int cov,
                                                    int64_t n, float* __restrict__ out) {
    const int64_t i = int64_t(blockIdx.x) * blockDim.x + threadIdx.x;
    if (i >= n) return;
    const int depth = site_info[(i / (33 * 34)) * 12 + 1 + which];
    const double sc = (cov > 0 && depth > cov) ? double(cov) / double(depth) : 1.0;
    out[i] = float(double(int(raw[i])) * sc);
}
}

extern "C" int cto_model_forward(cto_model* m, const float* x, int64_t B, float* logits, void* stream) {
    const int rc = forward_preamble("cto_model_forward", m, m && x && logits && B >= 0, B);
    if (rc != CTO_OK || B == 0) return rc;
    hipStream_t s = static_cast<hipStream_t>(stream);
    return m->kind == 1 ? bigru_forward(m, x, B, logits, s) : cvt_forward_timed(m, x, B, logits, s);
}

extern "C" int cto_model_forward_raw(cto_model* m, const int16_t* x_raw, const int32_t* site_info, int which, int min_rescale_cov, int64_t B,
                                     float* logits, void* stream) {
    const int rc = forward_preamble("cto_model_forward_raw", m, m && x_raw && site_info && logits && B >= 0 && (which == 0 || which == 1), B);
    if (rc != CTO_OK || B == 0) return rc;
    hipStream_t s = static_cast<hipStream_t>(stream);
    const bool native = m->kind == 1 ? !m->gw1_split : (m->fuse_blocks && m->fuse_embed && can_fuse_embed(m->st[0]));
    if (!native) {
        if (m->xexp_B < B) {
            if (m->b_xexp) (void)hipFree(m->b_xexp);
            m->b_xexp = nullptr; m->xexp_B = 0;
            CTO_HIP(hipMalloc(reinterpret_cast<void**>(&m->b_xexp), size_t(B) * 33 * 34 * sizeof(float)));
            m->xexp_B = B;
        }
        const int64_t n = B * 33 * 34;
        hipLaunchKernelGGL(k_expand_raw, dim3(unsigned(cdiv(n, 256))), dim3(256), 0, s, x_raw, site_info, which, min_rescale_cov, n, m->b_xexp);
        CTO_HIP(hipGetLastError());
        return cto_model_forward(m, m->b_xexp, B, logits, stream);
    }
    const RawIn raw{x_raw, site_info, which, min_rescale_cov};
    return m->kind == 1 ? bigru_forward(m, nullptr, B, logits, s, &raw) : cvt_forward_timed(m, nullptr, B, logits, s, &raw);
}

extern "C" int cto_model_profile(cto_model* m, int enable) {
    CTO_REQUIRE(m, CTO_EINVAL, "cto_model_profile: null model");
    m->prof = enable != 0;
    m->prof_all = enable == 2;
    m->prof_macs = m->kind == 1 ? int64_t(33) * 2 * 3 * 192 * (256 + 192) + int64_t(33) * 384 * 128 : m->macs;
    return CTO_OK;
}

extern "C" int cto_model_profile_read(cto_model* m, double* mean_ms, int64_t* macs_per_site);
static int profile_drain(std::vector<std::pair<hipEvent_t, hipEvent_t>>& evs, double* mean_ms) {
    double sum = 0.0;
    int n = 0;
    for (auto& e : evs) {
        CTO_HIP(hipEventSynchronize(e.second));
        float ms = 0.f;
        CTO_HIP(hipEventElapsedTime(&ms, e.first, e.second));
        sum += ms;
        ++n;
        (void)hipEventDestroy(e.first);
        (void)hipEventDestroy(e.second);
    }
    evs.clear();
    *mean_ms = n ? sum / n : 0.0;
    return n;
}

extern "C" int cto_model_profile_read_stage(cto_model* m, int stage, double* mean_ms, int64_t* macs_per_site) {
    CTO_REQUIRE(m && mean_ms && macs_per_site, CTO_EINVAL, "cto_model_profile_read_stage: null argument");
    if (stage == 0) return cto_model_profile_read(m, mean_ms, macs_per_site);
    CTO_REQUIRE(stage == 1 && m->kind == 1, CTO_EINVAL, "cto_model_profile_read_stage: stage 1 exists for the BiGRU only");
    *macs_per_site = int64_t(33) * 2 * 3 * 128 * (34 + 128);
    return profile_drain(m->prof_ev1, mean_ms);
}

extern "C" int cto_model_profile_read(cto_model* m, double* mean_ms, int64_t* macs_per_site) {
    CTO_REQUIRE(m && mean_ms && macs_per_site, CTO_EINVAL, "cto_model_profile_read: null argument");
    *macs_per_site = m->prof_macs;
    return profile_drain(m->prof_ev, mean_ms);
}

extern "C" int64_t cto_model_macs_per_site(const cto_model* m) { return m ? m->macs : 0; }
extern "C" int cto_model_n_out(const cto_model* m) { return m ? m->n_out : 0; }
extern "C" void cto_model_destroy(cto_model* m) { delete m; }
```

Before: 2.192 million sites/s.

## Run fused CvT stage-1 blocks on 16 waves and drop A double-buffering there

Templates the fused CvT block kernel on its wave count so a block can use 16 waves (1024 threads) instead of 8. GEMM tile ownership, the KV projection split, and the head prefetch/tail are generalized to spread M tiles across the extra waves. The 16-wave path is on by default only for stage 1 (C=16, not C=32) and turns off A-fragment double buffering to save registers. This trades more per-block parallelism on the small-channel stage for fewer blocks per CU and more barrier cost.

```diff
diff --git a/clairs_to_amd/csrc/cvt_block.h b/clairs_to_amd/csrc/cvt_block.h
--- a/clairs_to_amd/csrc/cvt_block.h
+++ b/clairs_to_amd/csrc/cvt_block.h
@@ -31,16 +31,15 @@
 template <int C, int W, int WKV, int TS>
 __host__ __device__ constexpr bool MT_EXACT() { return (TS * W) % 16 == 0 && (TS * WKV) % 16 == 0; }
 
-constexpr int CVT_BLOCK_THREADS = 512;
-constexpr int CVT_WAVES = CVT_BLOCK_THREADS / 64;
-
-template <int N>
+constexpr int CVT_WAVES = 8;
+
+template <int N, int NWAVES = CVT_WAVES>
 struct ColOwn {
     static constexpr int TILES = N / 16;
-    static constexpr int NOWN = TILES < CVT_WAVES ? TILES : CVT_WAVES;
-    static constexpr int MSPLIT = CVT_WAVES / NOWN;
+    static constexpr int NOWN = TILES < NWAVES ? TILES : NWAVES;
+    static constexpr int MSPLIT = NWAVES / NOWN;
     static constexpr int NTW = TILES / NOWN;
-    static_assert(TILES * 16 == N && CVT_WAVES % NOWN == 0 && NTW * NOWN == TILES, "unsupported GEMM width");
+    static_assert((NWAVES == 8 || NWAVES == 16) && TILES * 16 == N && NWAVES % NOWN == 0 && NTW * NOWN == TILES, "unsupported GEMM width");
 };
 template <int MTx, int MSPLIT>
 struct MSplit {
@@ -49,27 +48,27 @@
     static constexpr int LAST = MTx - FULL * MTG;
 };
 struct TileSpan { int tile0, mbase, mcount; };
-template <int N, int MTx>
+template <int N, int MTx, int NWAVES = CVT_WAVES>
 __device__ __forceinline__ TileSpan tile_span(int wave) {
-    using O = ColOwn<N>;
+    using O = ColOwn<N, NWAVES>;
     constexpr int MTG = MSplit<MTx, O::MSPLIT>::MTG;
     const int mb = (wave / O::NOWN) * MTG;
     const int left = MTx - mb;
     return TileSpan{(wave % O::NOWN) * O::NTW, mb, left < 0 ? 0 : (left > MTG ? MTG : left)};
 }
-template <int N, int MTx, int KCH>
-__device__ __forceinline__ void gemm_span(const TileSpan& sp, const float* A, int lda, const float* const (&wrow)[ColOwn<N>::NTW],
-                                          const BPre<ColOwn<N>::NTW>& pre,
-                                          f32x4 (&acc)[MSplit<MTx, ColOwn<N>::MSPLIT>::MTG][ColOwn<N>::NTW], int j, int kg) {
-    using S = MSplit<MTx, ColOwn<N>::MSPLIT>;
-    constexpr int NTW = ColOwn<N>::NTW;
+template <int N, int MTx, int KCH, int NWAVES = CVT_WAVES>
+__device__ __forceinline__ void gemm_span(const TileSpan& sp, const float* A, int lda, const float* const (&wrow)[ColOwn<N, NWAVES>::NTW],
+                                          const BPre<ColOwn<N, NWAVES>::NTW>& pre,
+                                          f32x4 (&acc)[MSplit<MTx, ColOwn<N, NWAVES>::MSPLIT>::MTG][ColOwn<N, NWAVES>::NTW], int j, int kg) {
+    using S = MSplit<MTx, ColOwn<N, NWAVES>::MSPLIT>;
+    constexpr int NTW = ColOwn<N, NWAVES>::NTW;
     const float* A0 = A + sp.mbase * 16 * lda;
-    if (ColOwn<N>::MSPLIT == 1 || sp.mcount == S::MTG) {
-        gemm_lds<S::MTG, NTW, KCH>(A0, lda, wrow, pre, acc, j, kg);
+    if (ColOwn<N, NWAVES>::MSPLIT == 1 || sp.mcount == S::MTG) {
+        gemm_lds<S::MTG, NTW, KCH, NWAVES == 8>(A0, lda, wrow, pre, acc, j, kg);
     } else if constexpr (S::LAST > 0) {
         if (sp.mcount == S::LAST) {
             f32x4 (&sub)[S::LAST][NTW] = reinterpret_cast<f32x4 (&)[S::LAST][NTW]>(acc);
-            gemm_lds<S::LAST, NTW, KCH>(A0, lda, wrow, pre, sub, j, kg);
+            gemm_lds<S::LAST, NTW, KCH, NWAVES == 8>(A0, lda, wrow, pre, sub, j, kg);
         }
     }
 }
@@ -92,31 +91,34 @@
     }
 }
 
-template <int C, int W, int WKV, int TS>
+template <int C, int W, int WKV, int TS, int NWAVES = CVT_WAVES>
 __host__ __device__ constexpr int cvt_blocks_per_cu() {
+    if (NWAVES == 16) return 1;
     return CvtBlockGeom<C, W, WKV, TS>::LDS_BYTES * 3 <= 160 * 1024 ? 3 : (CvtBlockGeom<C, W, WKV, TS>::LDS_BYTES * 2 <= 160 * 1024 ? 2 : 1);
 }
 
-template <int C, int W, int WKV, int TS, int CIN, bool HEAD, int SPLIT = 0>
-__global__ __launch_bounds__(CVT_BLOCK_THREADS, (2 * cvt_blocks_per_cu<C, W, WKV, TS>())) void k_cvt_block(float* __restrict__ h, CvtStageParams sp,
-                                                                                                            HeadTailParams hp, int heads, int B) {
+template <int C, int W, int WKV, int TS, int CIN, bool HEAD, int SPLIT = 0, int NWAVES = CVT_WAVES>
+__global__ __launch_bounds__(NWAVES * 64, (NWAVES / 4 * cvt_blocks_per_cu<C, W, WKV, TS, NWAVES>())) void k_cvt_block(float* __restrict__ h, CvtStageParams sp,
+                                                                                                                      HeadTailParams hp, int heads, int B) {
     using G = CvtBlockGeom<C, W, WKV, TS>;
     constexpr bool SP = SPLIT != 0, F16 = SPLIT == 1;
+    static_assert(!SP || NWAVES == CVT_WAVES, "split GEMMs: 8 waves");
     static_assert(!SP || (C % 64 == 0 && MT_EXACT<C, W, WKV, TS>()), "split GEMMs: 32-wide k chunks, 16-byte LayerNorm pieces, no pad rows");
     using WPtr = std::conditional_t<SP, const unsigned short*, const float*>;
     static_assert(CIN == 0 || G::emb_floats(CIN) <= G::ALIAS, "stage input tile does not fit the free LDS");
     static_assert(!HEAD || G::HEAD_OK, "classifier tail needs a 16-site tile and room for its scratch");
     static_assert(G::MT * 16 * G::RS <= G::TMP_FLOATS, "LayerNorm staging tile does not fit the q|k|v region");
-    constexpr int NT = CVT_BLOCK_THREADS, NWV = CVT_WAVES;
+    constexpr int NT = NWAVES * 64, NWV = NWAVES;
     constexpr int R = G::R, MT = G::MT, MTKV = G::MTKV, RKV = G::RKV, RS = G::RS, QS = G::QS, HC = G::HC, US = G::US;
     static_assert(C % 16 == 0 && C <= 128 && NT % C == 0, "channel count must be 16, 32, 64 or 128");
-    using OC = ColOwn<C>;
-    using OQ = ColOwn<64>;
-    using OKV = ColOwn<128>;
-    using OF = ColOwn<HC>;
+    using OC = ColOwn<C, NWV>;
+    using OQ = ColOwn<64, NWV>;
+    using OKV = ColOwn<128, NWV>;
+    using OF = ColOwn<HC, NWV>;
     constexpr int MGC = MSplit<MT, OC::MSPLIT>::MTG, MGQ = MSplit<MT, OQ::MSPLIT>::MTG, MGF = MSplit<MT, OF::MSPLIT>::MTG;
+    constexpr int MGKV = MSplit<MTKV, OKV::MSPLIT>::MTG;
     constexpr int NTC = OC::NTW, NTF = OF::NTW;
-    static_assert(OQ::NTW == 1 && OKV::NTW == 1 && OKV::MSPLIT == 1, "q / kv tiles: one column tile per wave");
+    static_assert(OQ::NTW == 1 && OKV::NTW == 1 && OKV::NOWN == 8, "q / kv tiles: one column tile per wave");
     extern __shared__ __attribute__((aligned(16))) float smem[];
     float* sy = smem + G::OFF_Y;
     float* sykv = smem + G::OFF_YKV;
@@ -127,7 +129,8 @@
     float* su = smem + G::OFF_YKV;
 
     const int tid = threadIdx.x, lane = tid & 63, wave = tid >> 6, j = lane & 15, kg = lane >> 4;
-    const TileSpan spc = tile_span<C, MT>(wave), spq = tile_span<64, MT>(wave), spf = tile_span<HC, MT>(wave);
+    const TileSpan spc = tile_span<C, MT, NWV>(wave), spq = tile_span<64, MT, NWV>(wave), spf = tile_span<HC, MT, NWV>(wave);
+    const TileSpan spkv = tile_span<128, MTKV, NWV>(wave);
     const int site0 = blockIdx.x * TS;
     const int nsite = min(TS, B - site0);
     const int rows_valid = nsite * W;
@@ -298,7 +301,7 @@
         for (int mt = 0; mt < MGC; ++mt)
 #pragma unroll
             for (int nt = 0; nt < NTC; ++nt) acc_e[mt][nt] = f32x4{0.f, 0.f, 0.f, 0.f};
-        gemm_span<C, MT, KE>(spc, smem + G::OFF_YKV, 2 * PS, we_r, pre_e, acc_e, j, kg);
+        gemm_span<C, MT, KE, NWV>(spc, smem + G::OFF_YKV, 2 * PS, we_r, pre_e, acc_e, j, kg);
 #pragma unroll
         for (int nt = 0; nt < NTC; ++nt) {
             const int col = (spc.tile0 + nt) * 16 + j;
@@ -411,14 +414,15 @@
     auto pre_q = prefetch_b<1, C / KD>(wq_r);
     for (int hh = 0; hh < heads; ++hh) {
         const int wn = wave & 3;
-        WPtr wkv1_r[1] = {frag(p.wkv, p.wkv_s, (wave < 4 ? 0 : inner / 16) + hh * 4 + wn, C / KD, 0)};
+        const bool wk = NWV == 8 ? wave < 4 : (wave & 4) == 0;
+        WPtr wkv1_r[1] = {frag(p.wkv, p.wkv_s, (wk ? 0 : inner / 16) + hh * 4 + wn, C / KD, 0)};
         const auto pre_kv1 = prefetch_b<1, C / KD>(wkv1_r);
         {
             f32x4 aq[MGQ][1];
 #pragma unroll
             for (int mt = 0; mt < MGQ; ++mt) aq[mt][0] = f32x4{0.f, 0.f, 0.f, 0.f};
             if constexpr (SP) gemm_span_split<64, MT, C / 32, F16>(spq, sy, RS, C, wq_r, pre_q, aq, j, kg);
-            else gemm_span<64, MT, C / 16>(spq, sy, RS, wq_r, pre_q, aq, j, kg);
+            else gemm_span<64, MT, C / 16, NWV>(spq, sy, RS, wq_r, pre_q, aq, j, kg);
 #pragma unroll
             for (int mt = 0; mt < MGQ; ++mt)
                 if (mt < spq.mcount) {
@@ -430,16 +434,27 @@
         o_rows(hh, wo_r);
         const auto pre_o = prefetch_b<NTC, 64 / KD>(wo_r);
         {
-            f32x4 akv1[MTKV][1];
-#pragma unroll
-            for (int mt = 0; mt < MTKV; ++mt) akv1[mt][0] = f32x4{0.f, 0.f, 0.f, 0.f};
-            if constexpr (SP) gemm_lds_split<MTKV, 1, C / 32, F16>(sykv, RS, C, wkv1_r, pre_kv1, akv1, j, kg);
-            else gemm_lds<MTKV, 1, C / 16>(sykv, RS, wkv1_r, pre_kv1, akv1, j, kg);
-            float* dst = wave < 4 ? sk : sv;
-#pragma unroll
-            for (int mt = 0; mt < MTKV; ++mt)
-#pragma unroll
-                for (int r = 0; r < 4; ++r) dst[(mt * 16 + 4 * kg + r) * QS + wn * 16 + j] = akv1[mt][0][r];
+            f32x4 akv1[MGKV][1];
+#pragma unroll
+            for (int mt = 0; mt < MGKV; ++mt) akv1[mt][0] = f32x4{0.f, 0.f, 0.f, 0.f};
+            if constexpr (OKV::MSPLIT == 1) {
+                if constexpr (SP) gemm_lds_split<MTKV, 1, C / 32, F16>(sykv, RS, C, wkv1_r, pre_kv1, akv1, j, kg);
+                else gemm_lds<MTKV, 1, C / 16>(sykv, RS, wkv1_r, pre_kv1, akv1, j, kg);
+                float* dst = wk ? sk : sv;
+#pragma unroll
+                for (int mt = 0; mt < MTKV; ++mt)
+#pragma unroll
+                    for (int r = 0; r < 4; ++r) dst[(mt * 16 + 4 * kg + r) * QS + wn * 16 + j] = akv1[mt][0][r];
+            } else {
+                gemm_span<128, MTKV, C / 16, NWV>(spkv, sykv, RS, wkv1_r, pre_kv1, akv1, j, kg);
+                float* dst = wk ? sk : sv;
+#pragma unroll
+                for (int mt = 0; mt < MGKV; ++mt)
+                    if (mt < spkv.mcount) {
+#pragma unroll
+                        for (int r = 0; r < 4; ++r) dst[((spkv.mbase + mt) * 16 + 4 * kg + r) * QS + wn * 16 + j] = akv1[mt][0][r];
+                    }
+            }
         }
         lds_barrier();
         stamp();
@@ -492,7 +507,7 @@
         lds_barrier();
         stamp();
         if constexpr (SP) gemm_span_split<C, MT, 2, F16>(spc, sq, QS, 64, wo_r, pre_o, acc_o, j, kg);
-        else gemm_span<C, MT, 4>(spc, sq, QS, wo_r, pre_o, acc_o, j, kg);
+        else gemm_span<C, MT, 4, NWV>(spc, sq, QS, wo_r, pre_o, acc_o, j, kg);
         lds_barrier();
         stamp();
     }
@@ -533,7 +548,7 @@
 #pragma unroll
                 for (int nt = 0; nt < NTF; ++nt) au[mt][nt] = f32x4{0.f, 0.f, 0.f, 0.f};
             if constexpr (SP) gemm_span_split<HC, MT, C / 32, F16>(spf, sy, RS, C, w1_r, pre_w1, au, j, kg);
-            else gemm_span<HC, MT, C / 16>(spf, sy, RS, w1_r, pre_w1, au, j, kg);
+            else gemm_span<HC, MT, C / 16, NWV>(spf, sy, RS, w1_r, pre_w1, au, j, kg);
             const int n0 = cc * HC + spf.tile0 * 16;
 #pragma unroll
             for (int nt = 0; nt < NTF; ++nt) {
@@ -560,7 +575,7 @@
         }
         lds_barrier();
         if constexpr (SP) gemm_span_split<C, MT, HC / 32, F16>(spc, su, US, HC, w2_r, pre_w2, acc_f, j, kg);
-        else gemm_span<C, MT, HC / 16>(spc, su, US, w2_r, pre_w2, acc_f, j, kg);
+        else gemm_span<C, MT, HC / 16, NWV>(spc, su, US, w2_r, pre_w2, acc_f, j, kg);
         if (cc + 1 < 4 * C / HC) lds_barrier();
         stamp();
     }
@@ -593,20 +608,25 @@
         constexpr int K1 = G::KCH1;
         float* t1 = smem + G::OFF_YKV + 64;
         float* t2 = t1 + 16 * HEAD_T1S;
-        const float* w1_r1[1] = {p.w1p + int64_t(wave) * (K1 * 256) + 4 * lane};
+        const bool fc1w = NWV == 8 || wave < 8;
+        const float* w1_r1[1] = {p.w1p + int64_t(fc1w ? wave : 0) * (K1 * 256) + 4 * lane};
         BGroup<1, 7> g0;
-        load_group<1, K1, 7, 256>(g0, w1_r1, 0);
+        HeadPreN<NWV == 8 ? 2 : 1> hpre;
+        if (fc1w) load_group<1, K1, 7, 256>(g0, w1_r1, 0);
+        else head_prefetch<NWV>(hpre, hp);
         lds_barrier();
         stamp();
-        f32x4 a1[2][1] = {{f32x4{0.f, 0.f, 0.f, 0.f}}, {f32x4{0.f, 0.f, 0.f, 0.f}}};
-        HeadPre hpre;
-        gemm_m1<1, K1, 7, 256>(sy, W * RS, w1_r1, g0, a1, j, kg, [&] { head_prefetch(hpre, hp); });
-        const float bv = p.b1h[wave * 16 + j];
-#pragma unroll
-        for (int r = 0; r < 4; ++r) t1[(4 * kg + r) * HEAD_T1S + wave * 16 + j] = selu_fast(a1[0][0][r] + a1[1][0][r] + bv);
+        if (fc1w) {
+            f32x4 a1[2][1] = {{f32x4{0.f, 0.f, 0.f, 0.f}}, {f32x4{0.f, 0.f, 0.f, 0.f}}};
+            gemm_m1<1, K1, 7, 256>(sy, W * RS, w1_r1, g0, a1, j, kg, [&] { if constexpr (NWV == 8) head_prefetch<NWV>(hpre, hp); });
+            if constexpr (NWV != 8) head_prefetch<NWV>(hpre, hp);
+            const float bv = p.b1h[wave * 16 + j];
+#pragma unroll
+            for (int r = 0; r < 4; ++r) t1[(4 * kg + r) * HEAD_T1S + wave * 16 + j] = selu_fast(a1[0][0][r] + a1[1][0][r] + bv);
+        }
         lds_barrier();
         stamp();
-        head_tail(t1, t2, hp, B, site0, nsite, hpre);
+        head_tail<NWV>(t1, t2, hp, B, site0, nsite, hpre);
     }
     stamp();
 }
diff --git a/clairs_to_amd/csrc/cvt_gemm.h b/clairs_to_amd/csrc/cvt_gemm.h
--- a/clairs_to_amd/csrc/cvt_gemm.h
+++ b/clairs_to_amd/csrc/cvt_gemm.h
@@ -41,7 +41,7 @@
     return p;
 }
 
-template <int MT, int NTW, int KCH>
+template <int MT, int NTW, int KCH, bool ADB = true>
 __device__ __forceinline__ void gemm_lds(const float* __restrict__ A, int lda, const float* const (&wrow)[NTW],
                                          const BPre<NTW>& pre, f32x4 (&acc)[MT][NTW], int j, int kg) {
 #if CTO_CVT_ABL == 1
@@ -50,19 +50,22 @@
     float4 Bq[3][NTW];
 #pragma unroll
     for (int nt = 0; nt < NTW; ++nt) { Bq[0][nt] = pre.b0[nt]; Bq[1][nt] = pre.b1[nt]; }
-    float4 a[2][MT];
+    float4 a[ADB ? 2 : 1][MT];
     const float* Arow = A + j * lda + 4 * kg;
-#pragma unroll
-    for (int mt = 0; mt < MT; ++mt) a[0][mt] = *reinterpret_cast<const float4*>(Arow + mt * 16 * lda);
+    if constexpr (ADB) {
+#pragma unroll
+        for (int mt = 0; mt < MT; ++mt) a[0][mt] = *reinterpret_cast<const float4*>(Arow + mt * 16 * lda);
+    }
 #pragma unroll
     for (int c = 0; c < KCH; ++c) {
         if (c + 2 < KCH) {
 #pragma unroll
             for (int nt = 0; nt < NTW; ++nt) Bq[(c + 2) % 3][nt] = ldg4(wrow[nt] + (c + 2) * FRAG_CS);
         }
-        if (c + 1 < KCH) {
-#pragma unroll
-            for (int mt = 0; mt < MT; ++mt) a[(c + 1) & 1][mt] = *reinterpret_cast<const float4*>(Arow + mt * 16 * lda + (c + 1) * 16);
+        if (ADB ? c + 1 < KCH : true) {
+#pragma unroll
+            for (int mt = 0; mt < MT; ++mt)
+                a[ADB ? (c + 1) & 1 : 0][mt] = *reinterpret_cast<const float4*>(Arow + mt * 16 * lda + (ADB ? c + 1 : c) * 16);
         }
         __builtin_amdgcn_sched_barrier(0);
 #pragma unroll
@@ -73,7 +76,7 @@
                 const float bv = e == 0 ? b4.x : (e == 1 ? b4.y : (e == 2 ? b4.z : b4.w));
 #pragma unroll
                 for (int mt = 0; mt < MT; ++mt) {
-                    const float4 a4 = a[c & 1][mt];
+                    const float4 a4 = a[ADB ? c & 1 : 0][mt];
                     const float av = e == 0 ? a4.x : (e == 1 ? a4.y : (e == 2 ? a4.z : a4.w));
                     acc[mt][nt] = mfma16(av, bv, acc[mt][nt]);
                 }
@@ -212,23 +215,33 @@
 __host__ __device__ constexpr int head_t2s(int K) { return K * 128 + 4; }
 __host__ __device__ constexpr int head_lds_floats(int K) { return 16 * HEAD_T1S + 16 * head_t2s(K); }
 
-struct HeadPre {
-    BGroup<2, 8> g[2];
-};
-__device__ __forceinline__ void head_prefetch(HeadPre& hpre, const HeadTailParams& hp) {
+template <int NG>
+struct HeadPreN {
+    BGroup<2, 8> g[NG];
+};
+using HeadPre = HeadPreN<2>;
+template <int NWAVES = 8>
+__device__ __forceinline__ void head_prefetch(HeadPreN<NWAVES == 8 ? 2 : 1>& hpre, const HeadTailParams& hp) {
     const int tid = threadIdx.x, lane = tid & 63, wave = tid >> 6;
-    const float* w0 = hp.w2 + int64_t(wave) * (8 * 256) + 4 * lane;
-#pragma unroll
-    for (int pi = 0; pi < 2; ++pi) {
+    const float* w0 = hp.w2 + int64_t(NWAVES == 8 ? wave : wave & 7) * (8 * 256) + 4 * lane;
+    if constexpr (NWAVES == 8) {
+#pragma unroll
+        for (int pi = 0; pi < 2; ++pi) {
+            const float* wr[2] = {w0 + pi * 2 * 128 * 128, w0 + (pi * 2 + 1) * 128 * 128};
+            load_group<2, 8, 8, 256>(hpre.g[pi], wr, 0);
+        }
+    } else {
+        const int pi = wave >> 3;
         const float* wr[2] = {w0 + pi * 2 * 128 * 128, w0 + (pi * 2 + 1) * 128 * 128};
-        load_group<2, 8, 8, 256>(hpre.g[pi], wr, 0);
-    }
-}
-
-template <int K>
+        load_group<2, 8, 8, 256>(hpre.g[0], wr, 0);
+    }
+}
+
+template <int K, int NWAVES = 8>
 __device__ __forceinline__ void head_tail_k(const float* t1, float* t2, const HeadTailParams& hp, int64_t B, int64_t site0,
-                                            int nsite, HeadPre& hpre) {
-    const int tid = threadIdx.x, lane = tid & 63, wave = tid >> 6, j = lane & 15, kg = lane >> 4;
+                                            int nsite, HeadPreN<NWAVES == 8 ? 2 : 1>& hpre) {
+    const int tid = threadIdx.x, lane = tid & 63, wave = NWAVES == 8 ? tid >> 6 : (tid >> 6) & 7, j = lane & 15, kg = lane >> 4;
+    const int half = NWAVES == 8 ? 0 : tid >> 9;
     constexpr int T2S = head_t2s(K);
     static_assert(K % 2 == 0 && K >= 4, "heads are processed in pairs; two pairs arrive prefetched");
     const float* wr[2];
@@ -237,16 +250,18 @@
     const float* Arow = t1 + j * HEAD_T1S + 4 * kg;
 #pragma unroll
     for (int pi = 0; pi < K / 2; ++pi) {
+        if (NWAVES != 8 && (pi & 1) != half) continue;
+        BGroup<2, 8>& gw = hpre.g[NWAVES == 8 ? (pi & 1) : 0];
         f32x4 acc[2][2];
 #pragma unroll
         for (int a = 0; a < 2; ++a)
 #pragma unroll
             for (int q = 0; q < 2; ++q) acc[a][q] = f32x4{0.f, 0.f, 0.f, 0.f};
-        mfma_group<2, 8, 8>(hpre.g[pi & 1], Arow, 0, acc);
+        mfma_group<2, 8, 8>(gw, Arow, 0, acc);
         __builtin_amdgcn_sched_barrier(0);
         if (pi + 2 < K / 2) {
             const float* wn[2] = {wr[0] + (pi + 2) * 2 * 128 * 128, wr[1] + (pi + 2) * 2 * 128 * 128};
-            load_group<2, 8, 8, 256>(hpre.g[pi & 1], wn, 0);
+            load_group<2, 8, 8, 256>(gw, wn, 0);
         }
 #pragma unroll
         for (int q = 0; q < 2; ++q) {
@@ -273,10 +288,11 @@
         if (part == 0 && site < nsite) hp.logits[(int64_t(hh) * B + site0 + site) * 2 + o] = selu_f(sum + hp.b3[hh * 2 + o]);
     }
 }
+template <int NWAVES = 8>
 __device__ __forceinline__ void head_tail(const float* t1, float* t2, const HeadTailParams& hp, int64_t B, int64_t site0,
-                                          int nsite, HeadPre& hpre) {
-    if (hp.K == 4) head_tail_k<4>(t1, t2, hp, B, site0, nsite, hpre);
-    else head_tail_k<6>(t1, t2, hp, B, site0, nsite, hpre);
+                                          int nsite, HeadPreN<NWAVES == 8 ? 2 : 1>& hpre) {
+    if (hp.K == 4) head_tail_k<4, NWAVES>(t1, t2, hp, B, site0, nsite, hpre);
+    else head_tail_k<6, NWAVES>(t1, t2, hp, B, site0, nsite, hpre);
 }
 
 __global__ __launch_bounds__(512) void k_head(const float* __restrict__ slabs, int S, int64_t slab_stride,
diff --git a/clairs_to_amd/csrc/models.hip b/clairs_to_amd/csrc/models.hip
--- a/clairs_to_amd/csrc/models.hip
+++ b/clairs_to_amd/csrc/models.hip
@@ -97,6 +97,7 @@
     bool fuse_blocks = true;
     bool fuse_embed = true;
     bool fuse_head = true;
+    int cvt_waves = 0;
     bool prof = false;
     bool prof_all = false;
     std::vector<std::pair<hipEvent_t, hipEvent_t>> prof_ev;
@@ -295,13 +296,13 @@
     int n_out = 0;
 };
 
-template <int C, int W, int WKV, int TS, int CIN, bool HEAD, int SPLIT = 0>
+template <int C, int W, int WKV, int TS, int CIN, bool HEAD, int SPLIT = 0, int NWAVES = CVT_WAVES>
 int launch_cvt_block(hipStream_t s, float* h, const BlockDev* blocks, int nblk, int heads, int64_t B, const BlockExtra& ex) {
     using G = CvtBlockGeom<C, W, WKV, TS>;
     static_assert(G::LDS_BYTES <= 160 * 1024, "fused CvT block does not fit the 160 KB LDS of a gfx950 CU");
     static bool attr_set = false;
     if (!attr_set) {
-        CTO_HIP(hipFuncSetAttribute(reinterpret_cast<const void*>(&k_cvt_block<C, W, WKV, TS, CIN, HEAD, SPLIT>),
+        CTO_HIP(hipFuncSetAttribute(reinterpret_cast<const void*>(&k_cvt_block<C, W, WKV, TS, CIN, HEAD, SPLIT, NWAVES>),
                                     hipFuncAttributeMaxDynamicSharedMemorySize, int(G::LDS_BYTES)));
         attr_set = true;
     }
@@ -335,37 +336,41 @@
         p.w1p = ex.head->w1p; p.b1h = ex.head->b1;
         hp = HeadTailParams{ex.head->w2, ex.head->b2, ex.head->w3, ex.head->b3, ex.logits, ex.n_out};
     }
-    hipLaunchKernelGGL((k_cvt_block<C, W, WKV, TS, CIN, HEAD, SPLIT>), dim3(unsigned(cdiv(B, TS))), dim3(CVT_BLOCK_THREADS), G::LDS_BYTES,
+    hipLaunchKernelGGL((k_cvt_block<C, W, WKV, TS, CIN, HEAD, SPLIT, NWAVES>), dim3(unsigned(cdiv(B, TS))), dim3(NWAVES * 64), G::LDS_BYTES,
                        s, h, sp, hp, heads, int(B));
     CTO_HIP(hipGetLastError());
     if (prof_on) {
         long long hst[256];
         CTO_HIP(hipStreamSynchronize(s));
         CTO_HIP(hipMemcpy(hst, prof_buf, sizeof(hst), hipMemcpyDeviceToHost));
-        fprintf(stderr, "k_cvt_block<%d,%d,%d,%d,%d,%d> x%d stamps:", C, W, WKV, TS, CIN, int(HEAD), nblk);
+        fprintf(stderr, "k_cvt_block<%d,%d,%d,%d,%d,%d> %d waves x%d stamps:", C, W, WKV, TS, CIN, int(HEAD), NWAVES, nblk);
         for (int i = 1; i < 256 && hst[i]; ++i) fprintf(stderr, " %lld", hst[i] - hst[i - 1]);
         fprintf(stderr, "\n");
     }
     return CTO_OK;
 }
 
-template <int C, int W, int WKV, int TS, int CIN, int SPLIT>
+template <int C, int W, int WKV, int TS, int CIN, int SPLIT, int NWAVES = CVT_WAVES>
 int dispatch_block_kind(hipStream_t s, float* h, const BlockDev* blocks, int nblk, int heads, int64_t B, const BlockExtra& ex, bool embed, bool head) {
     if constexpr (C == 128 && CvtBlockGeom<C, W, WKV, TS>::HEAD_OK) {
-        if (head) return embed ? launch_cvt_block<C, W, WKV, TS, CIN, true, SPLIT>(s, h, blocks, nblk, heads, B, ex)
-                               : launch_cvt_block<C, W, WKV, TS, 0, true, SPLIT>(s, h, blocks, nblk, heads, B, ex);
-    }
-    return embed ? launch_cvt_block<C, W, WKV, TS, CIN, false, SPLIT>(s, h, blocks, nblk, heads, B, ex)
-                 : launch_cvt_block<C, W, WKV, TS, 0, false, SPLIT>(s, h, blocks, nblk, heads, B, ex);
-}
-template <int C, int W, int WKV, int TS, int CIN>
+        if (head) return embed ? launch_cvt_block<C, W, WKV, TS, CIN, true, SPLIT, NWAVES>(s, h, blocks, nblk, heads, B, ex)
+                               : launch_cvt_block<C, W, WKV, TS, 0, true, SPLIT, NWAVES>(s, h, blocks, nblk, heads, B, ex);
+    }
+    return embed ? launch_cvt_block<C, W, WKV, TS, CIN, false, SPLIT, NWAVES>(s, h, blocks, nblk, heads, B, ex)
+                 : launch_cvt_block<C, W, WKV, TS, 0, false, SPLIT, NWAVES>(s, h, blocks, nblk, heads, B, ex);
+}
+template <int C, int W, int WKV, int TS, int CIN, int NWDEF>
 int dispatch_block(hipStream_t s, float* h, const BlockDev* blocks, int nblk, int heads, int64_t B, const BlockExtra& ex, bool embed, bool head,
-                   int split) {
+                   int split, int waves) {
+    static_assert(NWDEF == 8 || NWDEF == 16, "a fused CvT block runs on 8 or 16 waves");
     if constexpr (C % 64 == 0 && MT_EXACT<C, W, WKV, TS>()) {
         if (split == 1) return dispatch_block_kind<C, W, WKV, TS, CIN, 1>(s, h, blocks, nblk, heads, B, ex, embed, head);
         if (split == 2) return dispatch_block_kind<C, W, WKV, TS, CIN, 2>(s, h, blocks, nblk, heads, B, ex, embed, head);
     }
-    return dispatch_block_kind<C, W, WKV, TS, CIN, 0>(s, h, blocks, nblk, heads, B, ex, embed, head);
+    if constexpr (C != 32) {
+        if ((waves ? waves : NWDEF) == 16) return dispatch_block_kind<C, W, WKV, TS, CIN, 0, 16>(s, h, blocks, nblk, heads, B, ex, embed, head);
+    }
+    return dispatch_block_kind<C, W, WKV, TS, CIN, 0, 8>(s, h, blocks, nblk, heads, B, ex, embed, head);
 }
 #ifndef CTO_CVT_TS1
 #define CTO_CVT_TS1 8
@@ -376,6 +381,15 @@
 #ifndef CTO_CVT_TS3
 #define CTO_CVT_TS3 16
 #endif
+#ifndef CTO_CVT_NW1
+#define CTO_CVT_NW1 16
+#endif
+#ifndef CTO_CVT_NW2
+#define CTO_CVT_NW2 8
+#endif
+#ifndef CTO_CVT_NW3
+#define CTO_CVT_NW3 8
+#endif
 struct FusedGeom { int c, w, wkv, ts, cin; };
 const FusedGeom* fused_geom(const StageDev& st) {
     static const FusedGeom G[4] = {{128, 5, 3, CTO_CVT_TS3, 64}, {64, 9, 5, CTO_CVT_TS2, 16}, {16, 17, 9, CTO_CVT_TS1, 34}, {32, 17, 9, CTO_CVT_TS1, 34}};
@@ -387,13 +401,13 @@
 bool can_fuse_head(const StageDev& st, const HeadDev& hd) { const FusedGeom* g = fused_geom(st); return g && g->ts == 16 && g->c == 128 && hd.w1p; }
 
 int try_fused_blocks(hipStream_t s, const StageDev& st, const BlockDev* b, int nblk, float* h, int64_t B, const BlockExtra& ex, bool embed,
-                     bool head, int split) {
+                     bool head, int split, int waves) {
     int rc = CTO_OK;
     if (!b->wq_s) split = 0;
-    if (st.c == 128 && st.w == 5 && st.wkv == 3) rc = dispatch_block<128, 5, 3, CTO_CVT_TS3, 64>(s, h, b, nblk, st.heads, B, ex, embed, head, split);
-    else if (st.c == 64 && st.w == 9 && st.wkv == 5) rc = dispatch_block<64, 9, 5, CTO_CVT_TS2, 16>(s, h, b, nblk, st.heads, B, ex, embed, head, split);
-    else if (st.c == 16 && st.w == 17 && st.wkv == 9) rc = dispatch_block<16, 17, 9, CTO_CVT_TS1, 34>(s, h, b, nblk, st.heads, B, ex, embed, head, split);
-    else if (st.c == 32 && st.w == 17 && st.wkv == 9) rc = dispatch_block<32, 17, 9, CTO_CVT_TS1, 34>(s, h, b, nblk, st.heads, B, ex, embed, head, split);
+    if (st.c == 128 && st.w == 5 && st.wkv == 3) rc = dispatch_block<128, 5, 3, CTO_CVT_TS3, 64, CTO_CVT_NW3>(s, h, b, nblk, st.heads, B, ex, embed, head, split, waves);
+    else if (st.c == 64 && st.w == 9 && st.wkv == 5) rc = dispatch_block<64, 9, 5, CTO_CVT_TS2, 16, CTO_CVT_NW2>(s, h, b, nblk, st.heads, B, ex, embed, head, split, waves);
+    else if (st.c == 16 && st.w == 17 && st.wkv == 9) rc = dispatch_block<16, 17, 9, CTO_CVT_TS1, 34, CTO_CVT_NW1>(s, h, b, nblk, st.heads, B, ex, embed, head, split, waves);
+    else if (st.c == 32 && st.w == 17 && st.wkv == 9) rc = dispatch_block<32, 17, 9, CTO_CVT_TS1, 34, CTO_CVT_NW1>(s, h, b, nblk, st.heads, B, ex, embed, head, split, waves);
     else return 0;
     return rc == CTO_OK ? 1 : rc;
 }
@@ -427,7 +441,7 @@
                 const bool head = m->fuse_head && si == 2 && bi + size_t(nblk) == st.blocks.size() && can_fuse_head(st, m->head);
                 ex.xin = in; ex.st = &st; ex.head = &m->head; ex.logits = logits; ex.n_out = m->n_out;
                 ex.raw = (si == 0 && embed) ? raw : nullptr;
-                const int fr = try_fused_blocks(s, st, &b, nblk, hbuf, B, ex, embed, head, m->cvt_split);
+                const int fr = try_fused_blocks(s, st, &b, nblk, hbuf, B, ex, embed, head, m->cvt_split, m->cvt_waves);
                 if (fr < 0) return fr;
                 if (fr == 1) {
                     if (head) return CTO_OK;
@@ -793,6 +807,11 @@
     if (const char* e = getenv("CTO_CVT_UNFUSED")) m->fuse_blocks = !(e[0] == '1');
     if (const char* e = getenv("CTO_CVT_NO_EMBED_FUSE")) m->fuse_embed = !(e[0] == '1');
     if (const char* e = getenv("CTO_CVT_NO_HEAD_FUSE")) m->fuse_head = !(e[0] == '1');
+    if (const char* e = getenv("CTO_CVT_WAVES")) {
+        const std::string v(e);
+        CTO_REQUIRE(v == "8" || v == "16", CTO_EINVAL, "CTO_CVT_WAVES must be 8 or 16, not '%s'", e);
+        m->cvt_waves = v == "16" ? 16 : 8;
+    }
     *out = m.release();
     return CTO_OK;
 }
```

Result: no change. 2.200 million sites/s (median of 6 runs) (+0.4%).
